# ZKTLabs/zkt-plonk

Measured on AMD Instinct MI355X. Metric: proofs/sec (withdraw, n=2^20), higher is better.
Workload: dtype u32 limbs (256-bit Montgomery); 1 GPU; full prove, WithdrawCircuit INPUTS=8 HEIGHT=64 Poseidon x5 (1019498 gates, 538 Poseidon gadgets), bn254, n=2^20, TABLE_SIZE=1024, 12 public inputs; parallelism=proofs sharded across 1 GPU(s), chained=True, distinct_witnesses=2, witness_on_device=True, table_cached=True, proof_bytes=802

## Files before the change

include/zkt_plonk.h:

```cpp
#ifndef ZKT_PLONK_H
#define ZKT_PLONK_H

#include <stddef.h>
#include <stdint.h>

#ifdef __cplusplus
extern "C" {
#endif

typedef struct zkt_ctx zkt_ctx;

enum {
    ZKT_CURVE_BN254 = 0,
    ZKT_CURVE_BLS12_381 = 1
};

enum {
    ZKT_OK = 0,
    ZKT_ERR_INVALID_ARGUMENT = 1,
    ZKT_ERR_INVALID_DOMAIN_SIZE = 2,
    ZKT_ERR_HIP = 3,
    ZKT_ERR_NO_DEVICE = 4,
    ZKT_ERR_TOO_MANY_COEFFICIENTS = 5,
    ZKT_ERR_ZERO_DENOMINATOR = 6,
    ZKT_ERR_EQUAL_CHALLENGES = 7,
    ZKT_ERR_NOT_IN_TABLE = 8,
    ZKT_ERR_QUOTIENT_TOO_SHORT = 9,
    ZKT_ERR_NOT_LOADED = 10,
    ZKT_ERR_COMM = 11
};

int zkt_ctx_create(int curve_id, int device_id, zkt_ctx** out);
void zkt_ctx_destroy(zkt_ctx* ctx);
int zkt_ctx_fork(zkt_ctx* ctx, zkt_ctx** out);
const char* zkt_last_error(const zkt_ctx* ctx);
int zkt_ctx_set_stream(zkt_ctx* ctx, void* hip_stream);
int zkt_ctx_synchronize(zkt_ctx* ctx);
int zkt_profile_enable(zkt_ctx* ctx, int on);
int zkt_profile_get(zkt_ctx* ctx, const char* name, uint64_t* calls, double* total_ms);
const char* zkt_version(void);

typedef struct {
    void* user;
    int rank;
    int world;
    int device_buffers;
    int (*all_gather)(void* user, const void* send, void* recv, size_t bytes, int on_device, void* hip_stream);
    int (*all_gather_async)(void* user, const void* d_send, void* d_recv, size_t bytes, void* hip_stream);
} zkt_comm_vtable;
#define ZKT_QUOTIENT_CHUNKS 4
int zkt_ctx_set_comm(zkt_ctx* ctx, const zkt_comm_vtable* comm);
int zkt_shard_range(size_t total, int rank, int world, size_t* lo, size_t* hi);
int zkt_comm_stats(zkt_ctx* ctx, uint64_t* calls, uint64_t* bytes_sent);
int zkt_comm_selftest(const zkt_comm_vtable* comm, const void* send, void* recv, size_t bytes);

int zkt_dev_alloc(zkt_ctx* ctx, size_t bytes, void** dptr);
int zkt_dev_free(zkt_ctx* ctx, void* dptr);
int zkt_dev_upload(zkt_ctx* ctx, void* dptr, const void* host, size_t bytes);
int zkt_dev_download(zkt_ctx* ctx, void* host, const void* dptr, size_t bytes);

int zkt_ntt(zkt_ctx* ctx, int log_n, int inverse, int coset, const uint64_t* in, size_t in_len, uint64_t* out);
int zkt_ntt_dev(zkt_ctx* ctx, int log_n, int inverse, int coset, const void* d_in, size_t in_len, void* d_out);
int zkt_ntt_class(zkt_ctx* ctx, int log_n, int log_big, int cls, const uint64_t* in, size_t in_len, uint64_t* out);
int zkt_domain_group_gen(zkt_ctx* ctx, int log_n, uint64_t* out4);

int zkt_srs_load(zkt_ctx* ctx, const uint64_t* g1_xy_mont, size_t count);
int zkt_srs_load_dev(zkt_ctx* ctx, const void* d_g1_xy_mont, size_t count);
int zkt_srs_generate(zkt_ctx* ctx, const uint64_t* tau_canonical4, size_t count);
int zkt_srs_download(zkt_ctx* ctx, size_t offset, size_t count, uint64_t* out_xy_mont);
int zkt_srs_generate_g2(int curve_id, const uint64_t* tau_canonical4, uint64_t* out_h, uint64_t* out_beta_h);
int zkt_srs_load_slice(zkt_ctx* ctx, const uint64_t* g1_xy_mont_slice, size_t offset, size_t count, size_t total);
int zkt_srs_generate_slice(zkt_ctx* ctx, const uint64_t* tau_canonical4, size_t offset, size_t count, size_t total);
int zkt_msm_g1(zkt_ctx* ctx, const uint64_t* scalars, size_t len, size_t base_offset, int scalars_montgomery,
               uint64_t* out_xy_mont, int* out_is_infinity);
int zkt_msm_g1_dev(zkt_ctx* ctx, const void* d_scalars, size_t len, size_t base_offset, int scalars_montgomery,
                   void* out_xy_mont_host);
int zkt_msm_enqueue_dev(zkt_ctx* ctx, const void* d_scalars, size_t len, size_t base_offset, int scalars_montgomery);
int zkt_msm_info(zkt_ctx* ctx, int* window_bits, int* windows, size_t* srs_count);

#define ZKT_MSM_BASES_MAX ((size_t)1 << 22)
int zkt_msm_g1_bases(zkt_ctx* ctx, const uint64_t* bases_xy_mont, const uint64_t* scalars, size_t n,
                     int scalars_montgomery, uint64_t* out_xy_mont, int* out_is_infinity);
int zkt_msm_g1_bases_dev(zkt_ctx* ctx, const void* d_bases_xy_mont, const void* d_scalars, size_t n,
                         int scalars_montgomery, uint64_t* out_xy_mont_host, int* out_is_infinity);
int zkt_msm_bases_info(zkt_ctx* ctx, size_t n, int scalars_montgomery, int* window_bits, int* windows);

#define ZKT_KZG_BATCH_MAX 32
int zkt_kzg_commit_batch(zkt_ctx* ctx, const uint64_t* const* coeffs, const size_t* lens, int k,
                         int scalars_montgomery, uint64_t* out_xy_mont, int* out_is_infinity);
int zkt_kzg_commit_batch_dev(zkt_ctx* ctx, const void* const* d_coeffs, const size_t* lens, int k,
                             int scalars_montgomery, uint64_t* out_xy_mont, int* out_is_infinity);
int zkt_kzg_open(zkt_ctx* ctx, const uint64_t* const* coeffs, const size_t* lens, int k,
                 const uint64_t* challenges_mont, const uint64_t* point_mont,
                 uint64_t* out_w_xy_mont, int* out_w_is_infinity, uint64_t* out_evals_mont);
int zkt_kzg_open_dev(zkt_ctx* ctx, const void* const* d_coeffs, const size_t* lens, int k,
                     const uint64_t* challenges_mont, const uint64_t* point_mont,
                     uint64_t* out_w_xy_mont, int* out_w_is_infinity, uint64_t* out_evals_mont);

int zkt_ctx_set_lagrange(zkt_ctx* ctx, int on);
int zkt_ctx_set_wire_elimination(zkt_ctx* ctx, int mode);
int zkt_ctx_set_quotient_route(zkt_ctx* ctx, int mode);
int zkt_ctx_set_fused_passes(zkt_ctx* ctx, int mode);
int zkt_lagrange_info(zkt_ctx* ctx, int* log_n, size_t* bases);
int zkt_commit_evals_dev(zkt_ctx* ctx, const void* d_evals, const uint64_t* blinders, int k, int path, uint64_t* out_xy_mont,
                         int* out_is_infinity);

enum {
    ZKT_TRANSCRIPT_MERLIN = 0,
    ZKT_TRANSCRIPT_ETHEREUM = 1
};
typedef struct zkt_transcript zkt_transcript;
zkt_transcript* zkt_transcript_new(int kind, const char* label);
void zkt_transcript_free(zkt_transcript* t);
void zkt_transcript_append_u64(zkt_transcript* t, const char* label, uint64_t v);
void zkt_transcript_append_scalars(zkt_transcript* t, const char* label, const uint8_t* le32, size_t count, int single);
void zkt_transcript_append_commitment(zkt_transcript* t, const char* label, const uint8_t* x_le, const uint8_t* y_le,
                                      size_t fq_bytes, int is_infinity);
void zkt_transcript_challenge_scalar(zkt_transcript* t, const char* label, int fr_bits, uint8_t out_le32[32]);
void zkt_transcript_seed(zkt_transcript* t, uint64_t circuit_size, const uint8_t* xy_le, const uint8_t* is_infinity,
                         size_t fq_bytes);
int zkt_transcript_append_message(zkt_transcript* t, const char* label, const uint8_t* msg, size_t len);
int zkt_transcript_challenge_bytes(zkt_transcript* t, const char* label, uint8_t* out, size_t len);

typedef struct {
    void* user;
    void (*append_u64)(void* user, const char* label, uint64_t v);
    void (*append_scalars)(void* user, const char* label, const uint64_t* fr_mont, size_t count, int single);
    void (*append_commitment)(void* user, const char* label, const uint64_t* g1_xy_mont, int is_infinity);
    void (*challenge_scalar)(void* user, const char* label, uint64_t* fr_mont_out4);
} zkt_transcript_vtable;

int zkt_circuit_load(zkt_ctx* ctx, int log_n, const uint64_t* const* pk_polys, const size_t* pk_lens);

int zkt_circuit_setup(zkt_ctx* ctx, int log_n, const uint64_t* const* evals, const size_t* eval_lens, int evals_on_device,
                      uint64_t* out_commitments, int* out_is_infinity);

int zkt_circuit_sigma_dev(zkt_ctx* ctx, int log_n, const uint32_t* d_w_l, const uint32_t* d_w_r, const uint32_t* d_w_o,
                          size_t n_rows, size_t n_vars, void* const* d_sigma);
int zkt_circuit_setup_wiring(zkt_ctx* ctx, int log_n, const uint64_t* const* evals, const size_t* eval_lens,
                             int evals_on_device, const uint32_t* w_l, const uint32_t* w_r, const uint32_t* w_o,
                             size_t n_rows, size_t n_vars, int wiring_on_device,
                             uint64_t* out_commitments, int* out_is_infinity);

typedef struct {
    const uint64_t* a_evals;
    const uint64_t* b_evals;
    const uint64_t* c_evals;
    size_t n_rows;
    const uint64_t* table;
    size_t table_len;
    const size_t* pi_pos;
    const uint64_t* pi_vals;
    size_t n_pi;
    const uint64_t* blinders;
    int wires_on_device;
    const uint64_t* variables;
    size_t n_vars;
    const uint32_t* w_l;
    const uint32_t* w_r;
    const uint32_t* w_o;
} zkt_prove_inputs;
#define ZKT_VARIABLE_ZERO 0xFFFFFFFFu

int zkt_prove(zkt_ctx* ctx, const zkt_prove_inputs* in, zkt_transcript* transcript, uint8_t* proof_out,
              size_t proof_cap, size_t* proof_len);
int zkt_prove_set_next(zkt_ctx* ctx, const zkt_prove_inputs* next);
int zkt_prove_with(zkt_ctx* ctx, const zkt_prove_inputs* in, const zkt_transcript_vtable* transcript,
                   uint8_t* proof_out, size_t proof_cap, size_t* proof_len);

enum {
    ZKT_CHECK_WIRING = 1
};
#define ZKT_CHECK_NONE ((uint64_t)-1)
typedef struct {
    int satisfied;
    int checked;
    uint64_t n_arithmetic;
    uint64_t first_arithmetic;
    uint64_t residual[4];
    uint64_t n_lookup;
    uint64_t first_lookup;
    uint64_t n_wiring;
// ... 359 lines not shown
```

zkt-plonk_amd/_lib.py:

```python
from __future__ import annotations

import ctypes
import os
import re
from typing import Optional

import numpy as np

_HERE = os.path.dirname(os.path.abspath(__file__))
_LIB = os.environ.get("ZKT_LIB_PATH") or os.path.join(_HERE, "libzkt_plonk_hip.so")
_HEADER = os.path.join(_HERE, "..", "include", "zkt_plonk.h")

MSM_BASES_MAX = 1 << 22
G1_DECOMPRESS_MAX = 1 << 22
VERIFY_BATCH_DEV_MAX = MSM_BASES_MAX // 24
KZG_BATCH_MAX = 32
CURVE_BN254 = 0
CURVE_BLS12_381 = 1
_CURVES = {"bn254": 0, "bls12_381": 1, "bls12-381": 1, 0: 0, 1: 1}

_lib = None


class ZktError(RuntimeError):
# ... 1643 lines not shown

    def debug_verify_batch_tree(self, items, h_g2, beta_h_g2):
        ins, trs, k, h, bh, keep = _verify_batch_args(self.curve, items, h_g2, beta_h_g2)
        n_nodes = sum(verify_tree_levels(max(k, 1)))
        nodes = np.zeros((2, n_nodes, 2 * self.fq_limbs), dtype=np.uint64)
        inf = (ctypes.c_int * (2 * n_nodes))()
        rho = np.zeros((2 * max(k, 1), 4), dtype=np.uint64)
        self.check(self._L.zkt_debug_verify_batch_tree(self._h, ins, trs, k, u64p(h), u64p(bh), u64p(nodes), inf, u64p(rho)))
        return nodes, np.array([bool(x) for x in inf]).reshape(2, n_nodes), rho[:2 * k]

    def set_verify_terms(self, mode: int = 0):
        self._L.zkt_ctx_set_verify_terms.argtypes = [ctypes.c_void_p, ctypes.c_int]
        self.check(self._L.zkt_ctx_set_verify_terms(self._h, int(mode)))

    def debug_verify_terms(self, items, rho=None, forced=None, route: int = 2):
        rc, out = _verify_terms_call(self._L.zkt_debug_verify_terms, self._h, self.curve, items, rho, forced, route)
        self.check(rc)
        return out

    def msm_bases_info(self, n: int, montgomery: bool = True):
        c, w = ctypes.c_int(0), ctypes.c_int(0)
        self.check(self._L.zkt_msm_bases_info(self._h, n, int(montgomery), ctypes.byref(c), ctypes.byref(w)))
        return dict(window_bits=c.value, windows=w.value)

    def _kzg_polys(self, polys):
        arrs = [np.ascontiguousarray(p, dtype=np.uint64).reshape(-1, 4) for p in polys]
        ptrs = (ctypes.c_void_p * max(len(arrs), 1))(*[a.ctypes.data if a.shape[0] else None for a in arrs])
        return arrs, ptrs, self._kzg_lens([a.shape[0] for a in arrs])

    @staticmethod
    def _kzg_lens(lens):
        return (ctypes.c_size_t * max(len(lens), 1))(*[int(n) for n in lens])

    def _kzg_points(self, out, inf, k):
        W = 2 * self.fq_limbs
        return [(out[j * W:(j + 1) * W].copy(), bool(inf[j])) for j in range(k)]

    def kzg_commit_batch(self, polys, montgomery: bool = True):
        arrs, ptrs, lens = self._kzg_polys(polys)
        k = len(arrs)
        out = np.zeros(max(k, 1) * 2 * self.fq_limbs, dtype=np.uint64)
        inf = (ctypes.c_int * max(k, 1))()
        self.check(self._L.zkt_kzg_commit_batch(self._h, ptrs, lens, k, int(montgomery), u64p(out), inf))
        return self._kzg_points(out, inf, k)

    def kzg_commit_batch_dev(self, d_ptrs, lens, montgomery: bool = True):
        k = len(lens)
        ptrs = (ctypes.c_void_p * max(k, 1))(*[int(d) if d else None for d in d_ptrs])
        out = np.zeros(max(k, 1) * 2 * self.fq_limbs, dtype=np.uint64)
        inf = (ctypes.c_int * max(k, 1))()
        self.check(self._L.zkt_kzg_commit_batch_dev(self._h, ptrs, self._kzg_lens(lens), k, int(montgomery), u64p(out), inf))
        return self._kzg_points(out, inf, k)

    def _kzg_open_call(self, fn, ptrs, lens, k, challenges, z, evals):
        ch = np.ascontiguousarray(challenges, dtype=np.uint64).reshape(-1, 4)
        if ch.shape[0] != k:
            raise ValueError("kzg_open: %d polynomials, %d challenges" % (k, ch.shape[0]))
        zz = np.ascontiguousarray(z, dtype=np.uint64).reshape(4)
        w = np.zeros(2 * self.fq_limbs, dtype=np.uint64)
        inf = ctypes.c_int(0)
        ev = np.zeros((max(k, 1), 4), dtype=np.uint64)
        self.check(fn(self._h, ptrs, lens, k, u64p(ch) if k else None, u64p(zz), u64p(w), ctypes.byref(inf),
                      u64p(ev) if evals else None))
        return (w, bool(inf.value)), (ev[:k].copy() if evals else None)

    def kzg_open(self, polys, challenges, z, evals: bool = True):
        arrs, ptrs, lens = self._kzg_polys(polys)
        return self._kzg_open_call(self._L.zkt_kzg_open, ptrs, lens, len(arrs), challenges, z, evals)

    def kzg_open_dev(self, d_ptrs, lens, challenges, z, evals: bool = True):
        k = len(lens)
        ptrs = (ctypes.c_void_p * max(k, 1))(*[int(d) if d else None for d in d_ptrs])
        return self._kzg_open_call(self._L.zkt_kzg_open_dev, ptrs, self._kzg_lens(lens), k, challenges, z, evals)

    def msm_info(self):
        c, w, n = ctypes.c_int(0), ctypes.c_int(0), ctypes.c_size_t(0)
        self.check(self._L.zkt_msm_info(self._h, ctypes.byref(c), ctypes.byref(w), ctypes.byref(n)))
        return dict(window_bits=c.value, windows=w.value, srs_count=n.value)

    def set_lagrange(self, on: bool = True):
        self._L.zkt_ctx_set_lagrange.argtypes = [ctypes.c_void_p, ctypes.c_int]
        self.check(self._L.zkt_ctx_set_lagrange(self._h, int(on)))

    def set_wire_elimination(self, mode: int = 1):
        self._L.zkt_ctx_set_wire_elimination.argtypes = [ctypes.c_void_p, ctypes.c_int]
        self.check(self._L.zkt_ctx_set_wire_elimination(self._h, int(mode)))

    def lagrange_info(self):
        self._L.zkt_lagrange_info.argtypes = [ctypes.c_void_p, ctypes.POINTER(ctypes.c_int), ctypes.POINTER(ctypes.c_size_t)]
        lg, nb = ctypes.c_int(0), ctypes.c_size_t(0)
        self.check(self._L.zkt_lagrange_info(self._h, ctypes.byref(lg), ctypes.byref(nb)))
        return dict(log_n=lg.value, bases=nb.value)

    def commit_evals_dev(self, d_evals: int, blinders=None, path: int = 1):
        self._L.zkt_commit_evals_dev.argtypes = [ctypes.c_void_p, ctypes.c_void_p, ctypes.POINTER(ctypes.c_uint64), ctypes.c_int,
                                                 ctypes.c_int, ctypes.POINTER(ctypes.c_uint64), ctypes.POINTER(ctypes.c_int)]
        k = 0 if blinders is None else int(np.asarray(blinders).reshape(-1, 4).shape[0])
        bl = np.ascontiguousarray(blinders, dtype=np.uint64).reshape(-1, 4) if k else None
        out = np.zeros(2 * self.fq_limbs, dtype=np.uint64)
        inf = ctypes.c_int(0)
        self.check(self._L.zkt_commit_evals_dev(self._h, ctypes.c_void_p(d_evals), u64p(bl) if k else None, k, int(path),
                                                u64p(out), ctypes.byref(inf)))
        return out, bool(inf.value)

    def circuit_load(self, log_n: int, pk_polys):
        arrs = [np.ascontiguousarray(p, dtype=np.uint64).reshape(-1, 4) for p in pk_polys]
        assert len(arrs) == 10
        ptrs = (ctypes.POINTER(ctypes.c_uint64) * 10)(*[u64p(a) if a.size else ctypes.POINTER(ctypes.c_uint64)() for a in arrs])
        lens = (ctypes.c_size_t * 10)(*[a.shape[0] for a in arrs])
        self.check(self._L.zkt_circuit_load(self._h, log_n, ptrs, lens))
        self.circuit_log_n = log_n

    def circuit_setup(self, log_n: int, evals):
        arrs = [np.ascontiguousarray(p, dtype=np.uint64).reshape(-1, 4) for p in evals]
        assert len(arrs) == 10
        ptrs = (ctypes.POINTER(ctypes.c_uint64) * 10)(*[u64p(a) if a.size else ctypes.POINTER(ctypes.c_uint64)() for a in arrs])
        lens = (ctypes.c_size_t * 10)(*[a.shape[0] for a in arrs])
        out = np.zeros((10, 2 * self.fq_limbs), dtype=np.uint64)
        inf = (ctypes.c_int * 10)()
        self.check(self._L.zkt_circuit_setup(self._h, log_n, ptrs, lens, 0, u64p(out), inf))
        self.circuit_log_n = log_n
        return out, np.array([bool(x) for x in inf])

    def circuit_sigma(self, log_n: int, d_w_l: int, d_w_r: int, d_w_o: int, n_rows: int, n_vars: int, d_sigma=None):
        n = 1 << log_n if 0 <= log_n <= 25 else 0
        own = d_sigma is None
        if own:
            d_sigma = [self.alloc(max(n, 1) * 32) for _ in range(3)]
        try:
            ptrs = (ctypes.c_void_p * 3)(*d_sigma)
            self.check(self._L.zkt_circuit_sigma_dev(self._h, log_n, ctypes.c_void_p(d_w_l), ctypes.c_void_p(d_w_r),
                                                     ctypes.c_void_p(d_w_o), n_rows, n_vars, ptrs))
            return [self.download(p, (n, 4)) for p in d_sigma] if own else None
        finally:
            if own:
                for p in d_sigma:
                    self.free(p)

    def circuit_setup_wiring(self, log_n: int, evals, w_l, w_r, w_o, n_vars: int, n_rows: int = None):
        assert len(evals) == 10
        arrs = [np.zeros((0, 4), dtype=np.uint64) if p is None else np.ascontiguousarray(p, dtype=np.uint64).reshape(-1, 4)
                for p in evals]
        ptrs = (ctypes.POINTER(ctypes.c_uint64) * 10)(*[u64p(a) if a.size else ctypes.POINTER(ctypes.c_uint64)() for a in arrs])
        lens = (ctypes.c_size_t * 10)(*[a.shape[0] for a in arrs])
        on_device = isinstance(w_l, int)
        if on_device:
            assert n_rows is not None
            w = [ctypes.c_void_p(p) for p in (w_l, w_r, w_o)]
        else:
            idx = [np.ascontiguousarray(x, dtype=np.uint32).reshape(-1) for x in (w_l, w_r, w_o)]
            assert idx[0].shape == idx[1].shape == idx[2].shape
            n_rows = idx[0].shape[0] if n_rows is None else n_rows
            w = [x.ctypes.data_as(ctypes.c_void_p) if x.size else ctypes.c_void_p() for x in idx]
        out = np.zeros((10, 2 * self.fq_limbs), dtype=np.uint64)
        inf = (ctypes.c_int * 10)()
        self.check(self._L.zkt_circuit_setup_wiring(self._h, log_n, ptrs, lens, 0, w[0], w[1], w[2], n_rows, n_vars,
                                                    int(on_device), u64p(out), inf))
        self.circuit_log_n = log_n
        return out, np.array([bool(x) for x in inf])

    def _prepare(self, wires, n_rows, table, pi_pos, pi_vals, blinders, on_device, variables=None, idx=None, keep=()):
        table = np.ascontiguousarray(table, dtype=np.uint64).reshape(-1, 4)
        pi_vals = np.ascontiguousarray(pi_vals, dtype=np.uint64).reshape(-1, 4)
        if blinders is None:
            blinders = np.zeros((0, 4), dtype=np.uint64)
        else:
# ... 295 lines not shown
```

zkt-plonk_amd/csrc/capi.hip:

```cpp
#include "ctx.hpp"

#include <cstdlib>
#include "hostinv.hpp"
#include "ec.hpp"
#include "hostec.hpp"
#include "fx_test.hpp"
#include "msm.hpp"

#include <atomic>
#include <cstring>

namespace zkt {

const char* exp_env(const char* name) {
#ifdef ZKT_EXPERIMENTS
    return getenv(name);
#else
    (void)name;
    return nullptr;
#endif
}

int set_err(zkt_ctx* c, int code, const std::string& msg) {
    if (c) c->err = msg;
// ... 163 lines not shown
    (void)hipStreamSynchronize(c->stream);
    (void)hipDeviceSynchronize();
    for (auto& kv : c->prof) {
        for (auto& pr : kv.second.pending) {
            float ms = 0.f;
            if (hipEventElapsedTime(&ms, pr.first, pr.second) == hipSuccess) kv.second.total_ms += ms;
            c->event_pool.push_back(pr.first);
            c->event_pool.push_back(pr.second);
        }
        kv.second.pending.clear();
    }
}

template <class P>
__global__ void k_fr_mul(const Fe<P>* a, const Fe<P>* b, Fe<P>* o, size_t n) {
    size_t i = (size_t)blockIdx.x * blockDim.x + threadIdx.x;
    if (i < n) fe_store<P>(o + i, fe_mul<P>(fe_load<P>(a + i), fe_load<P>(b + i)));
}

template <class P>
__global__ void k_fx_test(int op, const uint32_t* in, size_t n, uint32_t* out) {
    constexpr int W = 4 * FxP<P>::L;
    size_t i = (size_t)blockIdx.x * blockDim.x + threadIdx.x;
    if (i < n) fx_test_op<P>(op, in + i * W, out + i * W);
}
template <class Q>
__global__ void k_xyzz_test(int op, const uint32_t* in, size_t n, uint32_t* out) {
    constexpr int W = 4 * FxP<Q>::L + 1;
    size_t i = (size_t)blockIdx.x * blockDim.x + threadIdx.x;
    if (i < n) xyzz_test_op<Q>(op, in + i * 2 * W, out + i * W);
}

template <class P>
static int dump_params(uint32_t* out, size_t words) {
    const int N = P::N;
    if (words < (size_t)(3 * N + 1)) return -1;
    for (int i = 0; i < N; ++i) out[i] = P::mod(i);
    out[N] = P::INV;
    for (int i = 0; i < N; ++i) out[N + 1 + i] = P::one(i);
    for (int i = 0; i < N; ++i) out[2 * N + 1 + i] = P::r2(i);
    return N;
}

}

using namespace zkt;

extern "C" {

const char* zkt_version(void) { return "zkt-plonk_amd 0.1 (gfx950)"; }

int zkt_ctx_create(int curve_id, int device_id, zkt_ctx** out) {
    if (!out) return ZKT_ERR_INVALID_ARGUMENT;
    *out = nullptr;
    if (curve_id != ZKT_CURVE_BN254 && curve_id != ZKT_CURVE_BLS12_381) return ZKT_ERR_INVALID_ARGUMENT;
    int count = 0;
    if (hipGetDeviceCount(&count) != hipSuccess || count <= 0 || device_id < 0 || device_id >= count)
        return ZKT_ERR_NO_DEVICE;
    if (hipSetDevice(device_id) != hipSuccess) return ZKT_ERR_NO_DEVICE;
    zkt_ctx* c = new zkt_ctx(device_id);
    c->batch_off = exp_env("ZKT_MSM_NO_BATCH") != nullptr;
    c->aux_off = exp_env("ZKT_NO_AUX") != nullptr;
    if (const char* parts = exp_env("ZKT_FUSED_PARTS")) c->fused_parts = atoi(parts) & 63;
    c->curve = curve_id;
    if (hipStreamCreateWithFlags(&c->stream, hipStreamNonBlocking) != hipSuccess) {
        delete c;
        return ZKT_ERR_HIP;
    }
    c->own_stream = true;
    *out = c;
    return ZKT_OK;
}

int zkt_ctx_fork(zkt_ctx* parent, zkt_ctx** out) {
    if (!parent || !out) return ZKT_ERR_INVALID_ARGUMENT;
    *out = nullptr;
    if (parent->sharded()) return set_err(parent, ZKT_ERR_INVALID_ARGUMENT, "zkt_ctx_fork: not for a context with a communicator");
    zkt_ctx* c = nullptr;
    int rc = zkt_ctx_create(parent->curve, parent->device, &c);
    if (rc) return rc;
    (void)hipStreamSynchronize(parent->stream);
    c->is_fork = true;
    c->lagrange_off = parent->lagrange_off;
    c->wire_elim_mode = parent->wire_elim_mode;
    c->quotient_route = parent->quotient_route;
    c->fused_passes = parent->fused_passes;
    c->verify_terms_mode = parent->verify_terms_mode;
    c->fused_parts = parent->fused_parts;
    c->batch_off = parent->batch_off;
    c->aux_off = parent->aux_off;
    c->ntt_plans = parent->ntt_plans;
    if ((rc = msm_fork(c, parent)) || (rc = circuit_fork(c, parent))) {
        parent->err = c->err;
        zkt_ctx_destroy(c);
        return rc;
    }
    *out = c;
    return ZKT_OK;
}

void zkt_ctx_destroy(zkt_ctx* c) {
    if (!c) return;
    (void)hipSetDevice(c->device);
    (void)hipStreamSynchronize(c->stream);
    circuit_release(c);
    msm_release(c);
    prof_resolve(c);
    for (hipEvent_t e : c->event_pool) (void)hipEventDestroy(e);
    c->event_pool.clear();
    c->msmb.reset();
    c->kzg.reset();
    c->ntt_plans.clear();
    if (c->comm.pinned) (void)hipHostFree(c->comm.pinned);
    c->owned.clear();
    if (c->own_stream && c->stream) (void)hipStreamDestroy(c->stream);
    delete c;
}

int zkt_ctx_set_comm(zkt_ctx* c, const zkt_comm_vtable* comm) {
    if (!c) return ZKT_ERR_INVALID_ARGUMENT;
    if (int rf = refuse_if_forked(c, "zkt_ctx_set_comm")) return rf;
    if (c->is_fork && comm && comm->world > 1) return set_err(c, ZKT_ERR_INVALID_ARGUMENT, "a forked context cannot take a communicator");
    if (comm && comm->world > 1) {
        const int w = comm->world;
        if ((w != 2 && w != 4 && w != 8) || comm->rank < 0 || comm->rank >= w || !comm->all_gather)
            return set_err(c, ZKT_ERR_INVALID_ARGUMENT, "communicator: world must be 1, 2, 4 or 8 with a valid rank and callback");
    }
    (void)hipSetDevice(c->device);
    (void)hipStreamSynchronize(c->stream);
    circuit_release(c);
    msm_release(c);
    c->comm.vt = zkt_comm_vtable{};
    c->comm.vt.world = 1;
    if (comm && comm->world > 1) c->comm.vt = *comm;
    c->comm.calls = 0;
    c->comm.bytes = 0;
    return ZKT_OK;
}
int zkt_shard_range(size_t total, int rank, int world, size_t* lo, size_t* hi) {
    if (world < 1 || rank < 0 || rank >= world || !lo || !hi) return ZKT_ERR_INVALID_ARGUMENT;
    const size_t base = total / (size_t)world, rem = total % (size_t)world;
    *lo = (size_t)rank * base + ((size_t)rank < rem ? (size_t)rank : rem);
    *hi = *lo + base + ((size_t)rank < rem ? 1 : 0);
    return ZKT_OK;
}
int zkt_comm_stats(zkt_ctx* c, uint64_t* calls, uint64_t* bytes_sent) {
    if (!c || !calls || !bytes_sent) return ZKT_ERR_INVALID_ARGUMENT;
    *calls = c->comm.calls;
    *bytes_sent = c->comm.bytes;
    return ZKT_OK;
}
int zkt_comm_selftest(const zkt_comm_vtable* comm, const void* send, void* recv, size_t bytes) {
    if (!comm || !comm->all_gather || !send || !recv) return ZKT_ERR_INVALID_ARGUMENT;
    return comm->all_gather(comm->user, send, recv, bytes, 0, nullptr) ? ZKT_ERR_COMM : ZKT_OK;
}

const char* zkt_last_error(const zkt_ctx* c) { return c ? c->err.c_str() : "null context"; }

int zkt_ctx_set_stream(zkt_ctx* c, void* hip_stream) {
    if (!c) return ZKT_ERR_INVALID_ARGUMENT;
    ZKT_HIP(c, hipStreamSynchronize(c->stream));
    if (c->own_stream && c->stream) (void)hipStreamDestroy(c->stream);
    c->stream = (hipStream_t)hip_stream;
    c->own_stream = false;
    return ZKT_OK;
}

int zkt_ctx_set_lagrange(zkt_ctx* c, int on) {
    if (!c) return ZKT_ERR_INVALID_ARGUMENT;
    c->lagrange_off = !on;
    ++c->msm_epoch;
    return ZKT_OK;
}

int zkt_ctx_set_wire_elimination(zkt_ctx* c, int mode) {
    if (!c) return ZKT_ERR_INVALID_ARGUMENT;
    if (mode < 0 || mode > 2) return set_err(c, ZKT_ERR_INVALID_ARGUMENT, "mode: 0 off, 1 automatic, 2 whenever a table can be built");
    c->wire_elim_mode = mode;
    ++c->msm_epoch;
    return ZKT_OK;
}

int zkt_ctx_set_quotient_route(zkt_ctx* c, int mode) {
    if (!c) return ZKT_ERR_INVALID_ARGUMENT;
    if (mode < 0 || mode > 2) return set_err(c, ZKT_ERR_INVALID_ARGUMENT, "mode: 0 automatic, 1 three classes, 2 the whole coset");
    c->quotient_route = mode;
    return ZKT_OK;
}

int zkt_ctx_set_fused_passes(zkt_ctx* c, int mode) {
    if (!c) return ZKT_ERR_INVALID_ARGUMENT;
    if (mode < 0 || mode > 2) return set_err(c, ZKT_ERR_INVALID_ARGUMENT, "mode: 0 automatic, 1 fused, 2 one launch per step");
    c->fused_passes = mode;
    return ZKT_OK;
}

int zkt_profile_enable(zkt_ctx* c, int on) {
    if (!c) return ZKT_ERR_INVALID_ARGUMENT;
    prof_resolve(c);
    if (on) c->prof.clear();
    c->prof_on = on == 2 ? 2 : (on != 0 ? 1 : 0);
    return ZKT_OK;
}
int zkt_profile_get(zkt_ctx* c, const char* name, uint64_t* calls, double* total_ms) {
    if (!c || !name || !calls || !total_ms) return ZKT_ERR_INVALID_ARGUMENT;
    prof_resolve(c);
    std::string key(name);
    const size_t hash = key.find("#launches");
    const bool want_launches = hash != std::string::npos;
    if (want_launches) key.resize(hash);
    auto it = c->prof.find(key);
    if (it == c->prof.end()) {
        *calls = 0;
        *total_ms = 0.0;
        return ZKT_OK;
    }
    *calls = want_launches ? it->second.launches : it->second.calls;
    *total_ms = it->second.total_ms;
    return ZKT_OK;
}

int zkt_ctx_synchronize(zkt_ctx* c) {
    if (!c) return ZKT_ERR_INVALID_ARGUMENT;
    ZKT_HIP(c, hipStreamSynchronize(c->stream));
    return ZKT_OK;
}

int zkt_dev_alloc(zkt_ctx* c, size_t bytes, void** dptr) {
    if (!c || !dptr) return ZKT_ERR_INVALID_ARGUMENT;
    (void)hipSetDevice(c->device);
    return dev_alloc(c, dptr, bytes);
}
int zkt_dev_free(zkt_ctx* c, void* dptr) {
    if (!c) return ZKT_ERR_INVALID_ARGUMENT;
    ZKT_HIP(c, hipStreamSynchronize(c->stream));
    dev_free(c, dptr);
    return ZKT_OK;
}
int zkt_dev_upload(zkt_ctx* c, void* dptr, const void* host, size_t bytes) {
    if (!c || (!dptr && bytes) || (!host && bytes)) return ZKT_ERR_INVALID_ARGUMENT;
    ZKT_HIP(c, hipMemcpyAsync(dptr, host, bytes, hipMemcpyHostToDevice, c->stream));
    ZKT_HIP(c, hipStreamSynchronize(c->stream));
    return ZKT_OK;
}
int zkt_dev_download(zkt_ctx* c, void* host, const void* dptr, size_t bytes) {
    if (!c || (!dptr && bytes) || (!host && bytes)) return ZKT_ERR_INVALID_ARGUMENT;
    ZKT_HIP(c, hipMemcpyAsync(host, dptr, bytes, hipMemcpyDeviceToHost, c->stream));
    ZKT_HIP(c, hipStreamSynchronize(c->stream));
    return ZKT_OK;
}

int zkt_ntt_dev(zkt_ctx* c, int log_n, int inverse, int coset, const void* d_in, size_t in_len, void* d_out) {
    if (!c || !d_out || (!d_in && in_len)) return set_err(c, ZKT_ERR_INVALID_ARGUMENT, "null pointer");
// ... 282 lines not shown
```

zkt-plonk_amd/csrc/circuit.hpp:

```cpp
#pragma once
#include "ctx.hpp"
#include "ec.hpp"
#include "hostinv.hpp"
#include "poly.hpp"
#include "quotient_classes.hpp"
#include <cstring>

namespace zkt {

enum { PK_QM = 0, PK_QL, PK_QR, PK_QO, PK_QC, PK_S1, PK_S2, PK_S3, PK_QLOOKUP, PK_QTABLE, PK_COUNT };
enum { CS_QM = 0, CS_QL, CS_QR, CS_QO, CS_QC, CS_QLOOKUP, CS_QTABLE, CS_S1, CS_S2, CS_S3, CS_X, CS_L1, CS_COUNT };
enum { W_A = 0, W_B, W_C, W_PI, W_Z1, W_Z2, W_T, W_H1, W_H2, W_COUNT };

struct CircuitKeys {
    std::shared_ptr<DevShared> keys_mem;
    void* pk[PK_COUNT] = {};
    size_t pk_len[PK_COUNT] = {};
    void* coset[CS_COUNT] = {};
    void* sigma_ev[3] = {};
    void* q_lookup_ev = nullptr;
    void* roots = nullptr;
    uint32_t zh_inv[4][8] = {};
};
struct ClassTables {
    std::shared_ptr<DevShared> class_mem;
    void* ccoset[CS_COUNT] = {};
    bool ccoset_ready = false;
    uint32_t key_win[4][QCW][8] = {};
    uint32_t qc_gamma[4][8] = {}, qc_vinv[9][8] = {}, qc_g3[3][8] = {};
};

struct CircuitState : CircuitKeys, ClassTables {
    DevSet work;
    explicit CircuitState(int device) : work(device) {}
    int log_n = 0;
    size_t n = 0;
    int G = 1, cls = 0, log_m = 0;
    size_t m = 0;
    void* wnext[4] = {};
    void* fold = nullptr;
    void* qgather = nullptr;
    bool have[16] = {};
    void* ev[8] = {};
    void* sc[4] = {};
    void* scan_tmp = nullptr;
    void* poly[13] = {};
    void* wcos[W_COUNT] = {};
    void* qev = nullptr;
    void* lag_scalars = nullptr;
    void* lag_scalars_q[3] = {};
    void* small = nullptr;
    uint32_t* status = nullptr;
    uint32_t* lk_u32 = nullptr;
    uint32_t lk_nkeys = 0;
    std::vector<uint32_t> lk_host_keys, lk_host_sorted, lk_host_counts, lk_host_order;
    bool has_next = false, prefetch_same_table = false;
    int prefetch_stage = 0;
    uint64_t prefetch_epoch = 0;
    zkt_prove_inputs next_in{}, prefetch_in{};
    void* poly_alt[3] = {};
    uint32_t* status_alt = nullptr;
    void* lk_keys = nullptr;
    size_t lk_cap = 0;
    void* pinned = nullptr;
    hipStream_t comm_stream = nullptr;
    hipEvent_t ev_piece[ZKT_QUOTIENT_CHUNKS] = {}, ev_gathered = nullptr;
    hipStream_t aux_stream = nullptr;
    hipEvent_t ev_aux_go = nullptr, ev_aux_done = nullptr;
    void* aux_scan_tmp = nullptr;
    void* aux_pw = nullptr;
    hipStream_t copy_stream = nullptr;
    hipEvent_t ev_copy[4] = {};
    void* pinned_pi = nullptr;
    uint32_t* pi_tab = nullptr;
    void* eval_pw = nullptr;
    std::vector<uint64_t> cached_table;
    bool t_cached = false, t_coset_valid = false;
    uint64_t t_srs_generation = 0;
    uint64_t t_commit_xy[12] = {};
    bool wire_route[3] = {};
    bool wire_dense_only = false;
    int wire_elim_force = -1;
    bool use_classes = false;
    void* heads = nullptr;
    void* d_win = nullptr;
    void* pinned_win = nullptr;
    hipEvent_t ev_win = nullptr;
    bool vk_cached = false;
    uint64_t vk_srs_generation = 0;
    uint64_t vk_commits[10 * 12] = {};
    int vk_inf[10] = {};
    size_t vk_table_size = 0;
    uint32_t last_u[6][8] = {};
    bool last_u_valid = false;
};

template <class P>
struct HostF {
    using F = Fe<P>;
    static F from_words(const uint64_t* w) {
        F r;
        memcpy(r.v, w, 32);
        return r;
    }
    static void to_le_bytes(const F& mont, uint8_t out[32]) {
        F c = fe_from_mont<P>(mont);
        memcpy(out, c.v, 32);
    }
    static F from_le_bytes(const uint8_t in[32]) {
        F c;
        memcpy(c.v, in, 32);
        return fe_to_mont<P>(c);
    }
};

template <class Q>
static void fq_to_le(const Fe<Q>& mont, uint8_t* out) {
    Fe<Q> c = fe_from_mont<Q>(mont);
    memcpy(out, c.v, Q::N * 4);
}

template <class Fn>
static auto by_curve(int curve, Fn&& f) {
    return curve == ZKT_CURVE_BN254 ? f(Bn254Curve{}) : f(Bls381Curve{});
}

enum : unsigned {
    ENTRY_DOMAIN = 1u,
    ENTRY_SRS = 2u,
    ENTRY_WHOLE_KEY = 4u,
    ENTRY_WHOLE_COSET = 8u,
    ENTRY_NO_NEXT = 16u,
    ENTRY_DEVICE = 32u,
    ENTRY_WITHDRAW = 64u,
    ENTRY_WORK = ENTRY_WHOLE_COSET | ENTRY_NO_NEXT | ENTRY_DEVICE | ENTRY_WITHDRAW,
};
inline int circuit_entry(zkt_ctx* c, unsigned needs, const char* who = "") {
    if (!c->circuit)
        return set_err(c, ZKT_ERR_NOT_LOADED, needs & ENTRY_DOMAIN ? "no circuit loaded (the domain comes from it)" : "no circuit loaded (zkt_circuit_load)");
    if ((needs & ENTRY_SRS) && !c->msm) return set_err(c, ZKT_ERR_NOT_LOADED, "no SRS loaded (zkt_srs_load)");
    if ((needs & ENTRY_WHOLE_KEY) && c->sharded()) return set_err(c, ZKT_ERR_INVALID_ARGUMENT, "not available on a sharded key");
    if ((needs & ENTRY_WHOLE_COSET) && (c->sharded() || c->circuit->G != 1))
        return set_err(c, ZKT_ERR_INVALID_ARGUMENT, std::string(who) + ": a sharded context holds one class of every coset and a slice of the key; use an unsharded one");
    if ((needs & ENTRY_NO_NEXT) && c->circuit->has_next) return set_err(c, ZKT_ERR_INVALID_ARGUMENT, std::string(who) + ": a next proof is announced");
    if (needs & ENTRY_DEVICE) (void)hipSetDevice(c->device);
    if (needs & ENTRY_WITHDRAW) c->circuit->prefetch_stage = 0;
    return ZKT_OK;
}

int circuit_key_coset(zkt_ctx* c, CircuitState& S, const void* poly, size_t len, void* out);
int circuit_commit_keys(zkt_ctx* c, CircuitState& S, const size_t* lens, uint64_t* out_commitments, int* out_is_inf);
int circuit_key_lens(zkt_ctx* c, const CircuitState& S, size_t* lens10);
int check_sharded_key(zkt_ctx* c);

template <class R>
static void circuit_zh4(int log_n, Fe<R> out[4]) {
    const size_t n = (size_t)1 << log_n;
    const Fe<R> one = fe_one<R>(), g = fe_from_u32<R>(R::GENERATOR), w4n = root_of_unity<R>(log_n + 2);
    const Fe<R> w4 = fe_pow_u64<R>(w4n, (uint64_t)n);
    Fe<R> cur = fe_pow_u64<R>(g, (uint64_t)n);
    for (int j = 0; j < 4; ++j) {
        out[j] = fe_sub<R>(cur, one);
        cur = fe_mul<R>(cur, w4);
// ... 38 lines not shown
```

zkt-plonk_amd/csrc/circuit_steps.hip:

```cpp
#include "circuit.hpp"
#include "msm.hpp"

namespace zkt {

template <class R>
static void debug_quotient_classes_host_t(int log_n, const uint64_t* windows, const uint64_t* challenges, uint64_t* out_u,
                                          uint64_t* out_consts) {
    typedef Fe<R> F;
    const QuotientClassConsts<R> q = quotient_class_consts<R>(log_n);
    for (int k = 0; k < 4; ++k) memcpy(out_consts + 4 * k, q.gamma[k].v, 32);
    for (int k = 0; k < 9; ++k) memcpy(out_consts + 4 * (4 + k), q.vinv[k].v, 32);
    for (int k = 0; k < 3; ++k) memcpy(out_consts + 4 * (13 + k), q.g3[k].v, 32);
    const uint32_t* w = (const uint32_t*)windows;
    QuotientWindows W{};
    const uint32_t** slot[10] = {&W.a, &W.b, &W.c, &W.z1, &W.z2, &W.t, &W.sigma1, &W.sigma2, &W.sigma3, &W.q_lookup};
    for (int k = 0; k < 10; ++k) *slot[k] = w + (size_t)k * QCW * 8;
    F alpha, beta, delta, u[6];
    memcpy(alpha.v, challenges, 32);
    memcpy(beta.v, challenges + 4, 32);
    memcpy(delta.v, challenges + 8, 32);
    quotient_top_coefficients<R>(log_n, W, alpha, beta, delta, u);
    for (int e = 0; e < 6; ++e) memcpy(out_u + 4 * e, u[e].v, 32);
}

}

using namespace zkt;

extern "C" {

int zkt_debug_quotient_top(zkt_ctx* c, uint64_t* out_u, int* out_on_classes) {
    if (!c || !out_u) return set_err(c, ZKT_ERR_INVALID_ARGUMENT, "null pointer");
    if (int rc = circuit_entry(c, 0)) return rc;
    const CircuitState& S = *c->circuit;
    if (out_on_classes) *out_on_classes = S.use_classes ? 1 : 0;
    memcpy(out_u, S.last_u, sizeof(S.last_u));
    return ZKT_OK;
}

int zkt_debug_quotient_coeffs(zkt_ctx* c, uint64_t* out, size_t count) {
    if (!c || !out) return set_err(c, ZKT_ERR_INVALID_ARGUMENT, "null pointer");
    if (int rc = circuit_entry(c, ENTRY_DEVICE)) return rc;
    const CircuitState& S = *c->circuit;
    if (count > 4 * S.n) return set_err(c, ZKT_ERR_INVALID_ARGUMENT, "the quotient vector holds 4n elements");
    ZKT_HIP(c, hipStreamSynchronize(c->stream));
    ZKT_HIP(c, hipMemcpy(out, S.qev, count * 32, hipMemcpyDeviceToHost));
    return ZKT_OK;
}

int zkt_debug_quotient_classes_host(int curve, int log_n, const uint64_t* windows, const uint64_t* challenges, uint64_t* out_u,
                                    uint64_t* out_consts) {
    if (!windows || !challenges || !out_u || !out_consts) return ZKT_ERR_INVALID_ARGUMENT;
    if (curve != ZKT_CURVE_BN254 && curve != ZKT_CURVE_BLS12_381) return ZKT_ERR_INVALID_ARGUMENT;
    return by_curve(curve, [&](auto C) {
        using R = typename decltype(C)::Fr;
        if (log_n < 3 || log_n + 2 > R::TWO_ADICITY) return (int)ZKT_ERR_INVALID_DOMAIN_SIZE;
        debug_quotient_classes_host_t<R>(log_n, windows, challenges, out_u, out_consts);
        return (int)ZKT_OK;
    });
}

int zkt_lagrange_info(zkt_ctx* c, int* log_n, size_t* bases) {
    if (!c) return ZKT_ERR_INVALID_ARGUMENT;
    const bool ready = c->circuit && lagrange_ready(c, c->circuit->log_n) && !c->lagrange_off;
    if (log_n) *log_n = ready ? c->circuit->log_n : -1;
    if (bases) *bases = ready ? lagrange_bases(c) : 0;
    return ZKT_OK;
}

int zkt_commit_evals_dev(zkt_ctx* c, const void* d_evals, const uint64_t* blinders, int k, int path, uint64_t* out_xy,
                         int* out_is_infinity) {
    if (!c || !d_evals || !out_xy || (k > 0 && !blinders)) return set_err(c, ZKT_ERR_INVALID_ARGUMENT, "null pointer");
    if (k < 0 || k > 3) return set_err(c, ZKT_ERR_INVALID_ARGUMENT, "0 .. 3 blinders");
    if (int rc0 = circuit_entry(c, ENTRY_DOMAIN | ENTRY_SRS | ENTRY_WHOLE_KEY | ENTRY_DEVICE | ENTRY_WITHDRAW)) return rc0;
    CircuitState& S = *c->circuit;
    const size_t n = S.n;
    int rc;
    if (path == 1) {
        if ((rc = lagrange_ensure(c, S.log_n))) return rc;
        if (!lagrange_ready(c, S.log_n)) return set_err(c, ZKT_ERR_NOT_LOADED, "the key is too short for the Lagrange-basis table");
    } else if (path != 0) {
        return set_err(c, ZKT_ERR_INVALID_ARGUMENT, "path: 0 coefficients, 1 Lagrange basis");
    }
    uint32_t* d_len = S.status + 8 + 12;
    void* d_bl = (char*)S.lag_scalars + (n + 8) * 32;
    void* poly = S.poly[12];
    ZKT_HIP(c, hipMemsetAsync(d_len, 0, 4, c->stream));
    if (k) ZKT_HIP(c, hipMemcpyAsync(d_bl, blinders, (size_t)k * 32, hipMemcpyHostToDevice, c->stream));
    if ((rc = ntt_run(c, S.log_n, 1, 0, d_evals, n, poly))) return rc;
    if (c->fused(4)) {
        const TrimBlindSpec tb{poly, d_bl, d_len, k};
        if ((rc = poly_trim_blind(c, &tb, 1, n, 8))) return rc;
    } else {
        if ((rc = poly_trim_len(c, poly, n, d_len, (char*)poly + n * 32, 8))) return rc;
        if (k && (rc = poly_add_blinders(c, poly, d_len, d_bl, k, n + 8))) return rc;
    }
    if (path == 0) return msm_g1_dev(c, poly, n + (size_t)k, 0, 1, out_xy, out_is_infinity);
    if ((rc = lagrange_scalars(c, d_evals, n, d_len, d_bl, k, S.roots, S.lag_scalars))) return rc;
    if ((rc = msm_begin(c, S.lag_scalars, n + (size_t)k, 0, 1, 0, 1))) return rc;
    uint64_t xy[12] = {};
    if ((rc = msm_end(c, 0, xy))) return rc;
    const size_t words = c->curve == ZKT_CURVE_BN254 ? 8 : 12;
    memcpy(out_xy, xy, words * 8);
    if (out_is_infinity) {
        bool any = false;
        for (size_t i = 0; i < words; ++i) any = any || xy[i] != 0;
        *out_is_infinity = any ? 0 : 1;
    }
    return ZKT_OK;
}

int zkt_debug_quotient(zkt_ctx* c, const uint64_t* challenges, const uint64_t* const* wit, const uint64_t* pi_pos,
                       const uint64_t* pi_vals, size_t n_pi, uint64_t* out) {
    if (!c || !challenges || !wit || !out || (n_pi && (!pi_pos || !pi_vals)))
        return set_err(c, ZKT_ERR_INVALID_ARGUMENT, "null pointer");
    if (int rc0 = circuit_entry(c, ENTRY_DEVICE)) return rc0;
    CircuitState& S = *c->circuit;
    if (S.G != 1) return set_err(c, ZKT_ERR_INVALID_ARGUMENT, "zkt_debug_quotient: whole-coset circuits only");
    if (n_pi > (size_t)QUOTIENT_PI_DIRECT_MAX) return set_err(c, ZKT_ERR_INVALID_ARGUMENT, "too many direct public inputs");
    for (size_t i = 0; i < n_pi; ++i)
        if (pi_pos[i] >= S.n) return set_err(c, ZKT_ERR_INVALID_ARGUMENT, "public input position out of range");
    const size_t bytes = 4 * S.n * 32;
    DevSet tmp(c->device);
    void* d[W_COUNT] = {};
    void* d_out = nullptr;
    uint32_t* d_tab = nullptr;
    int rc = ZKT_OK;
    for (int k = 0; k < W_COUNT && !rc; ++k) {
        if (k == W_PI && n_pi) continue;
        if (!wit[k]) rc = set_err(c, ZKT_ERR_INVALID_ARGUMENT, "null witness coset");
        else if (!(rc = tmp.alloc(c, &d[k], bytes)) && hipMemcpy(d[k], wit[k], bytes, hipMemcpyHostToDevice) != hipSuccess)
            rc = set_err(c, ZKT_ERR_HIP, "copy of a witness coset failed");
    }
    if (!rc) rc = tmp.alloc(c, &d_out, bytes);
    if (!rc && n_pi) {
        std::vector<uint32_t> tab(10 * n_pi);
        by_curve(c->curve, [&](auto C) { pi_rows<typename decltype(C)::Fr>(pi_pos, pi_vals, n_pi, 1, tab.data()); });
        if (!(rc = tmp.alloc(c, (void**)&d_tab, tab.size() * 4)) &&
            hipMemcpy(d_tab, tab.data(), tab.size() * 4, hipMemcpyHostToDevice) != hipSuccess)
            rc = set_err(c, ZKT_ERR_HIP, "copy of the public-input rows failed");
    }
    if (!rc) {
        QuotientArgs q = quotient_args(S, d, challenges, challenges + 4, challenges + 8, challenges + 12, challenges + 16);
        q.out = d_out;
        q.n4 = 4 * S.n;
        q.pi_tab = n_pi ? d_tab : nullptr;
        q.n_pi_direct = (uint32_t)n_pi;
        rc = quotient_pointwise(c, q);
        if (!rc && hipStreamSynchronize(c->stream) != hipSuccess) rc = set_err(c, ZKT_ERR_HIP, "quotient kernel failed");
        if (!rc && hipMemcpy(out, d_out, bytes, hipMemcpyDeviceToHost) != hipSuccess) rc = set_err(c, ZKT_ERR_HIP, "copy back failed");
    }
    return rc;
}

int zkt_debug_eval_lincomb(zkt_ctx* c, const uint64_t* const* polys, const size_t* lens, int k, const uint64_t* points,
                           const uint64_t* scalars, uint64_t* out_evals, uint64_t* out_lincomb, size_t out_len) {
    if (!c || !polys || !lens || !points || !scalars || !out_evals || !out_lincomb) return set_err(c, ZKT_ERR_INVALID_ARGUMENT, "null pointer");
    if (int rc0 = circuit_entry(c, ENTRY_DEVICE | ENTRY_WITHDRAW)) return rc0;
    CircuitState& S = *c->circuit;
    const size_t cap = S.n + 8;
    if (k < 1 || k > 12 || out_len < 1 || out_len > cap) return set_err(c, ZKT_ERR_INVALID_ARGUMENT, "1 .. 12 polynomials, out_len <= n + 8");
    for (int j = 0; j < k; ++j)
        if (!polys[j] || lens[j] < 1 || lens[j] > cap) return set_err(c, ZKT_ERR_INVALID_ARGUMENT, "1 .. n + 8 coefficients each");
    EvalArgs ea{};
    LinCombArgs lc{};
    ea.count = k;
    lc.nterms = k;
    for (int j = 0; j < k; ++j) {
        ZKT_HIP(c, hipMemcpyAsync(S.poly[j], polys[j], lens[j] * 32, hipMemcpyHostToDevice, c->stream));
        ea.poly[j] = lc.poly[j] = S.poly[j];
        ea.len[j] = lc.len[j] = lens[j];
        memcpy(ea.point[j], points + 4 * j, 32);
        memcpy(lc.scalar[j], scalars + 4 * j, 32);
    }
    void* d_partials = (char*)S.small + 64 * 32;
    void* d_results = (char*)S.small + 32 * 32;
    int rc = poly_eval_many(c, ea, d_partials, d_results, S.eval_pw);
    if (rc) return rc;
    if ((rc = poly_lincomb(c, lc, S.sc[0], out_len))) return rc;
    ZKT_HIP(c, hipMemcpyAsync(out_evals, d_results, (size_t)k * 32, hipMemcpyDeviceToHost, c->stream));
    ZKT_HIP(c, hipMemcpyAsync(out_lincomb, S.sc[0], out_len * 32, hipMemcpyDeviceToHost, c->stream));
    ZKT_HIP(c, hipStreamSynchronize(c->stream));
    return ZKT_OK;
}
// ... 25 lines not shown
```

zkt-plonk_amd/csrc/ctx.hpp:

```cpp
#pragma once
#include <hip/hip_runtime.h>
#include <stdint.h>
#include <stddef.h>
#include <map>
#include <string>
#include <tuple>
#include <vector>
#include <memory>

#include "../../include/zkt_plonk.h"
#include "fp.hpp"
#include "fx.hpp"
#include "ntt.hpp"

namespace zkt {

struct MsmState;
struct MsmBasesState;
struct KzgState;
struct CircuitState;

struct DevSet {
    const int device;
    std::vector<std::pair<void*, size_t>> mem;
    std::vector<void*> host;
    std::vector<hipStream_t> streams;
    std::vector<hipEvent_t> events;
    explicit DevSet(int dev) : device(dev) {}
    DevSet(const DevSet&) = delete;
    DevSet& operator=(const DevSet&) = delete;
    ~DevSet() { clear(); }
    void clear();
    int alloc(zkt_ctx* c, void** p, size_t bytes);
    void release(void* p);
    int pinned(zkt_ctx* c, void** p, size_t bytes, unsigned flags = 0);
    int stream(zkt_ctx* c, hipStream_t* s);
    int event(zkt_ctx* c, hipEvent_t* e);
};
struct DevBuf {
    void* p = nullptr;
    size_t bytes = 0;
};

}

struct zkt_ctx {
    int curve = 0;
    const int device;
    explicit zkt_ctx(int dev) : device(dev), owned(dev) {}
    hipStream_t stream = nullptr;
    bool own_stream = false;
    std::string err;

    std::map<std::tuple<int, int, int, int>, std::shared_ptr<void>> ntt_plans;
    int ntt_split_npass = 0;
    int ntt_split_log_r[3] = {0, 0, 0};
    zkt::DevBuf ntt_scratch, io_a, io_b;
    zkt::DevBuf check_scratch;
    zkt::DevBuf verify_scratch;

    int prof_on = 0;
    struct ProfSlot {
        std::vector<std::pair<hipEvent_t, hipEvent_t>> pending;
        double total_ms = 0.0;
        uint64_t calls = 0;
        uint64_t launches = 0;
    };
    std::map<std::string, ProfSlot> prof;
    std::vector<hipEvent_t> event_pool;

    struct Comm {
        zkt_comm_vtable vt{};
        void* pinned = nullptr;
        size_t pinned_bytes = 0;
        uint64_t calls = 0, bytes = 0;
    } comm;
    bool sharded() const { return comm.vt.world > 1; }

    std::shared_ptr<zkt::MsmState> msm;
    std::shared_ptr<zkt::MsmBasesState> msmb;
    std::shared_ptr<zkt::KzgState> kzg;
    size_t srs_check_chunk = 0;
    size_t store_chunk = 0;
    uint64_t msm_epoch = 0;
    uint64_t srs_generation = 0;
    bool is_fork = false;
    bool aux_off = false;
    bool batch_off = false;
    bool lagrange_off = false;
    int wire_elim_mode = 1;
    int quotient_route = 0;
    int verify_terms_mode = 0;
    int fused_passes = 0;
    int fused_parts = 63;
    bool fused(int part) const { return fused_passes != 2 && (fused_parts & part); }
    std::shared_ptr<zkt::CircuitState> circuit;
    zkt::DevSet owned;
};

namespace zkt {

const char* exp_env(const char* name);

int set_err(zkt_ctx* c, int code, const std::string& msg);
int refuse_if_forked(zkt_ctx* c, const char* what);
int hip_fail(zkt_ctx* c, hipError_t e, const char* what);

#define ZKT_HIP(c, call)                                        \
    do {                                                        \
        hipError_t _e = (call);                                 \
        if (_e != hipSuccess) return zkt::hip_fail((c), _e, #call); \
    } while (0)

struct ProfScope {
    zkt_ctx* c;
    zkt_ctx::ProfSlot* slot = nullptr;
    hipEvent_t e0 = nullptr, e1 = nullptr;
    hipStream_t stream = nullptr;
    uint64_t count = 1;
    ProfScope(zkt_ctx* ctx, const char* name, hipStream_t on_stream = nullptr, uint64_t units = 1);
    ~ProfScope();
};

int comm_all_gather_host(zkt_ctx* c, const void* send, void* recv, size_t bytes);
int comm_all_gather_dev(zkt_ctx* c, const void* d_send, void* d_recv, size_t bytes);
bool comm_async_available(const zkt_ctx* c);
int comm_all_gather_async(zkt_ctx* c, const void* d_send, void* d_recv, size_t bytes, hipStream_t st);

int grow(zkt_ctx* c, DevBuf& b, size_t bytes, DevSet* in = nullptr);
inline int dev_alloc(zkt_ctx* c, void** p, size_t bytes) { return c->owned.alloc(c, p, bytes); }
inline void dev_free(zkt_ctx* c, void* p) { c->owned.release(p); }

struct DevShared : DevSet {
    using DevSet::DevSet;
    std::shared_ptr<DevShared> from;
};
inline std::shared_ptr<DevShared> dev_shared_reader(const std::shared_ptr<DevShared>& of) {
    if (!of) return nullptr;
    auto r = std::make_shared<DevShared>(of->device);
    r->from = of;
    return r;
}
inline bool dev_shared_has_readers(const std::shared_ptr<DevShared>& m) { return m && m.use_count() > 1; }

template <class P>
Fe<P> root_of_unity(int log_n);
int ntt_run(zkt_ctx* c, int log_n, int inverse, int coset, const void* d_in, size_t in_len, void* d_out);
int ntt_run_batch(zkt_ctx* c, int log_n, int inverse, int coset, int nb, const void* const* d_in, const size_t* in_len,
                  void* const* d_out, const void* d_head = nullptr);
int ntt_fold_heads(zkt_ctx* c, int nb, const void* const* d_in, size_t n, const uint32_t* gammas, void* d_out);
int ntt_run_classes(zkt_ctx* c, int log_n, int inverse, const int codes[3], int nb, const void* const* d_in, const size_t* in_len,
                    void* const* d_out, size_t in_stride, size_t out_stride, const void* d_head = nullptr);
int ntt_class_code(int log_big, int cls);
int ntt_force_split(zkt_ctx* c, int npass, const int* log_r);
int ntt_run_class(zkt_ctx* c, int log_n, int log_big, int cls, const void* d_in, size_t in_len, void* d_out, void* d_fold);

void circuit_release(zkt_ctx* c);
int circuit_fork(zkt_ctx* child, const zkt_ctx* parent);
bool circuit_tables_have_readers(const zkt_ctx* c);

}
```

zkt-plonk_amd/csrc/msm.hip:

```cpp
#include "ctx.hpp"
#include "ec.hpp"
#include "ecx.hpp"
#include "hostec.hpp"
#include "msm.hpp"

#include <algorithm>
#include <functional>
#include <type_traits>
#include <cstdlib>
#include <cstring>

namespace zkt {

template <class C>
__global__ void k_srs_generate(Affine<typename C::Fq>* out, size_t count, Fe<typename C::Fr> tau_mont,
                               Affine<typename C::Fq> g, size_t first) {
    using Q = typename C::Fq;
    using R = typename C::Fr;
    size_t i = (size_t)blockIdx.x * blockDim.x + threadIdx.x;
    if (i >= count) return;
    Fe<R> s = fe_from_mont<R>(fe_from_mont<R>(fe_pow_u64<R>(tau_mont, (uint64_t)(first + i))));
    Xyzz<Q> acc = xyzz_identity<Q>();
    bool started = false;
#pragma unroll 1
// ... 720 lines not shown
    Xyzz<Q>* buckets = (Xyzz<Q>*)tb.buckets[blockIdx.y];
    const uint32_t* heavy = tb.heavy[blockIdx.y];
    const uint32_t chunk = tb.params[blockIdx.y][0];
    __shared__ Xyzz<Q> wsum[4];
    const uint32_t nheavy = heavy[0];
    const uint32_t base = offsets[1];
    for (uint32_t h = blockIdx.x; h < nheavy; h += gridDim.x) {
        const uint32_t b = heavy[1 + h];
        const uint32_t s = offsets[b], e = offsets[b + 1];
        const uint32_t t0 = (s - base) / chunk, t1 = (e - 1 - base) / chunk;
        XyzzX<Q> acc = xx_identity<Q>();
        for (uint32_t t = t0 + threadIdx.x; t <= t1; t += 256) acc = xx_add<Q, MSM_TAIL_INL>(acc, xx_load_raw<Q>(pieces + (size_t)t + b));
        acc = block_sum_256<Q, MSM_TAIL_INL>(acc, wsum);
        if (threadIdx.x == 0) xx_store<Q>(buckets + b, acc);
    }
}

template <class Q, bool MSM_TAIL_INL>
ZKT_D XyzzX<Q> wave_sum(XyzzX<Q> acc) {
#pragma unroll 1
    for (int d = 32; d >= 1; d >>= 1) {
        XyzzX<Q> o = xx_shfl_down<Q>(acc, d);
        if ((threadIdx.x & 63) + d >= 64) o = xx_identity<Q>();
        acc = xx_add<Q, MSM_TAIL_INL>(acc, o);
    }
    return acc;
}

struct MsmTailWindows {
    struct Strided {
        char* base;
        size_t stride;
        __device__ void* operator[](uint32_t y) const { return base + (size_t)y * stride; }
    };
    Strided buckets, rowcol, partials;
};

template <class C, bool MSM_TAIL_INL, class TB = MsmTailBatch>
__global__ __launch_bounds__(256) void k_msm_rowcol(uint32_t q1, uint32_t q2, TB tb) {
    using Q = typename C::Fq;
    const Xyzz<Q>* buckets = (const Xyzz<Q>*)tb.buckets[blockIdx.y];
    Xyzz<Q>* rc = (Xyzz<Q>*)tb.rowcol[blockIdx.y];
    const uint32_t NI = 1u << q1, NJ = 1u << q2;
    const uint32_t lane = threadIdx.x & 63u;
    const uint32_t w = blockIdx.x * 4u + (threadIdx.x >> 6);
    if (w >= NI + NJ) return;
    XyzzX<Q> acc = xx_identity<Q>();
    if (w < NI) {
        for (uint32_t j = lane; j < NJ; j += 64) acc = xx_add<Q, MSM_TAIL_INL>(acc, xx_load<Q>(buckets + (size_t)w * NJ + j));
    } else {
        const uint32_t j = w - NI;
        for (uint32_t i = lane; i < NI; i += 64) acc = xx_add<Q, MSM_TAIL_INL>(acc, xx_load<Q>(buckets + (size_t)i * NJ + j));
    }
    acc = wave_sum<Q, MSM_TAIL_INL>(acc);
    if (lane == 0) xx_store<Q>(rc + w, acc);
}

template <class C, bool MSM_TAIL_INL, class TB = MsmTailBatch>
__global__ __launch_bounds__(64) void k_msm_weighted_rows(uint32_t q1, uint32_t q2, uint32_t B, TB tb) {
    using Q = typename C::Fq;
    const Xyzz<Q>* rc = (const Xyzz<Q>*)tb.rowcol[blockIdx.y];
    const Xyzz<Q>* top_bucket = (const Xyzz<Q>*)tb.buckets[blockIdx.y] + B;
    Xyzz<Q>* partials = (Xyzz<Q>*)tb.partials[blockIdx.y];
    const uint32_t NI = 1u << q1, NJ = 1u << q2;
    const uint32_t lane = threadIdx.x & 63u;
    const uint32_t y = blockIdx.x;
    XyzzX<Q> acc = xx_identity<Q>();
    if (y == q1 + q2) {
        if (lane == 0) acc = xx_load<Q>(top_bucket);
    } else {
        const bool col = y < q2;
        const uint32_t k = col ? y : y - q2, low = (1u << k) - 1u;
        const uint32_t cnt = (col ? NJ : NI) >> 1;
        const Xyzz<Q>* src = col ? rc + NI : rc;
        for (uint32_t q = lane; q < cnt; q += 64) {
            const uint32_t idx = ((q & ~low) << 1) | (1u << k) | (q & low);
            acc = xx_add<Q, MSM_TAIL_INL>(acc, xx_load<Q>(src + idx));
        }
    }
    acc = wave_sum<Q, MSM_TAIL_INL>(acc);
    if (lane == 0) xx_store_ark<Q>(partials + y, acc);
}

template <class C>
__global__ void k_srs_to_fx(Affine<typename C::Fq>* table, size_t total) {
    using Q = typename C::Fq;
    size_t i = (size_t)blockIdx.x * blockDim.x + threadIdx.x;
    if (i >= total) return;
    Affine<Q> a = aff_load<Q>(table + i);
    if (aff_is_inf<Q>(a)) return;
    a.x = fx_pack<Q>(fx_cond_sub_p<Q>(fx_from_ark<Q>(a.x)));
    a.y = fx_pack<Q>(fx_cond_sub_p<Q>(fx_from_ark<Q>(a.y)));
    aff_store<Q>(table + i, a);
}

static int msm_rows(int c) { return c - 1; }

template <class C, bool VB = false>
static auto msm_pick_bin_count(int dig) -> decltype(&k_msm_bin_count<C, 0, VB>) {
    if constexpr (VB) {
        return k_msm_bin_count<C, 0, true>;
    } else {
        switch (dig) {
            case 1: return k_msm_bin_count<C, 1>;
            case 2: return k_msm_bin_count<C, 2>;
            case 3: return k_msm_bin_count<C, 3>;
            case 4: return k_msm_bin_count<C, 4>;
            case 5: return k_msm_bin_count<C, 5>;
            default: return k_msm_bin_count<C, 0>;
        }
    }
}
template <class C, class PF, bool VB = false>
static auto msm_pick_bin_scatter(int dig) -> decltype(&k_msm_bin_scatter<C, PF, 0, VB>) {
    if constexpr (VB) {
        return k_msm_bin_scatter<C, PF, 0, true>;
    } else {
        switch (dig) {
            case 1: return k_msm_bin_scatter<C, PF, 1>;
            case 2: return k_msm_bin_scatter<C, PF, 2>;
            case 3: return k_msm_bin_scatter<C, PF, 3>;
            case 4: return k_msm_bin_scatter<C, PF, 4>;
            case 5: return k_msm_bin_scatter<C, PF, 5>;
            default: return k_msm_bin_scatter<C, PF, 0>;
        }
    }
}

static int floor_log2(size_t x) {
    int l = 0;
    while ((x >> (l + 1)) != 0) ++l;
    return l;
}

static int msm_plan(zkt_ctx* c, int total, int cb, size_t points, bool own_buckets, MsmPlan& P) {
    P = MsmPlan{};
    const int W = (total + cb - 1) / cb;
    if (W > (int)sizeof(P.win.width)) return set_err(c, ZKT_ERR_INVALID_ARGUMENT, "msm_g1_bases: too many windows");
    const int lo = total / W, rem = total % W;
    P.W = P.win.W = W;
    int pos = 0;
    for (int w = 0; w < W; ++w) {
        P.win.width[w] = (uint8_t)(lo + (w < rem ? 1 : 0));
        P.win.start[w] = (uint16_t)pos;
        pos += P.win.width[w];
    }
    P.c = lo + (rem ? 1 : 0);
    P.dig = own_buckets ? 0 : msm_digit_layout(P.win, total);
    P.Bw = 1u << (P.c - 1);
    P.keys = own_buckets ? (uint32_t)W * P.Bw : P.Bw;
    const size_t m = (size_t)W * points;
    if (!own_buckets && m >= ((size_t)1 << 31))
        return set_err(c, ZKT_ERR_INVALID_ARGUMENT, "SRS too large for 31-bit table indices");
    {
        const size_t idx_max = (own_buckets ? points : m) - 1;
        int idx_bits = 1;
        while (idx_max >> idx_bits) ++idx_bits;
        int lb = 31 - idx_bits;
        if (lb > MSM_BIN_LB_MAX) lb = MSM_BIN_LB_MAX;
        P.packed = lb >= 4 && ((P.keys >> lb) + 1) < (uint32_t)MSM_MAX_NB1;
        P.lb = P.packed ? (uint32_t)lb : (uint32_t)MSM_BIN_LB_MAX;
        if (!P.packed && ((P.keys >> P.lb) + 1) >= (uint32_t)MSM_MAX_NB1) {
            P.lb = MSM_BIN_LB_WIDE;
            P.lcols = MSM_BIN_LB_WIDE;
        }
    }
    P.nb1 = (P.keys >> P.lb) + 1;
    if (P.nb1 >= (uint32_t)MSM_MAX_NB1 || m >= ((size_t)1 << 31))
        return set_err(c, ZKT_ERR_INVALID_ARGUMENT,
                       own_buckets ? "msm_g1_bases: digit layout outside the sort's range" : "msm: too many level-1 bins");
    P.l1_scalars = ((uint32_t)MSM_L1_CAP / (uint32_t)W) & ~63u;
    if (P.l1_scalars > 1024u) P.l1_scalars = 1024u;
    P.l2_items = (uint32_t)(m / MSM_L2_TILE + P.nb1);
    return ZKT_OK;
}

template <class C, bool VB>
static int msm_scatter_lds_cap(zkt_ctx* c, bool packed, int dig) {
    const int lds = (int)(((3 * (uint32_t)MSM_MAX_NB1 + 3) & ~3u) * 4 + MSM_L1_CAP * (packed ? 4 : 8));
// ... 35 lines not shown
    auto st = std::make_shared<MsmState>(c->device);
    struct Drain {
        zkt_ctx* c;
        ~Drain() { if (!c->msm) (void)hipStreamSynchronize(c->stream); }
    } drain{c};
    st->count = count;
    int lg = floor_log2(count ? count : 1);
    int cb = lg - 2;
    if (cb < 8) cb = 8;
    if (lg <= 20) {
        if (cb > 18) cb = 18;
        if (Q::N == 12) {
            if (lg == 20) cb = 19;
            else if (lg == 19) cb = 18;
            else if (lg == 17) cb = 16;
        } else if (lg >= 17) {
            cb = 17;
        }
    } else if (cb > 20) {
        cb = 20;
    }
    if (const char* e = exp_env("ZKT_MSM_CBITS")) {
        const int f = atoi(e);
        if (f >= 8 && f <= MSM_MAX_Y) cb = f;
    }
    int rc = msm_plan(c, R::BITS + 1, cb, count, false, st->plan);
    if (rc) return rc;
    const MsmPlan& P = st->plan;
    if (share) {
        st->table = share->table;
        st->table_mem = dev_shared_reader(share->table_mem);
        static_cast<LagrangeTable&>(*st) = *share;
        st->lag_mem = dev_shared_reader(share->lag_mem);
        if (share->wb.built && !share->wb.stale) {
            st->wb = share->wb;
            st->wb.mem = dev_shared_reader(share->wb.mem);
        }
        st->slice_off = share->slice_off;
        st->total = share->total;
    } else {
        st->table_mem = std::make_shared<DevShared>(c->device);
        if ((rc = st->table_mem->alloc(c, &st->table, (size_t)P.W * count * sizeof(Affine<Q>)))) return rc;
    }
    size_t m = (size_t)P.W * count;
    constexpr size_t NB = MSM_BATCH;
    auto up = [](size_t x) { return (x + 63) & ~(size_t)63; };
    st->strides.s_vals = up(m);
    st->strides.s_pairs_bytes = up(m) * 8;
    if ((rc = st->work.alloc(c, (void**)&st->vals2, NB * st->strides.s_vals * 4))) return rc;
    if ((rc = st->work.alloc(c, &st->pairs, NB * st->strides.s_pairs_bytes))) return rc;
    const size_t max_blk = (count + P.l1_scalars - 1) / P.l1_scalars;
    st->strides.s_bin_offs = up((size_t)P.nb1 * max_blk + 1);
    st->strides.s_bin_aux = up((size_t)P.nb1 * max_blk / MSM_SCAN_TILE + 4);
    st->strides.s_bin = up((size_t)P.nb1 + 1);
    st->strides.s_tile_desc = up(P.l2_items);
    st->strides.s_cnt = up((size_t)P.l2_items << P.lcols);
    if ((rc = st->work.alloc(c, (void**)&st->bin_offs, NB * st->strides.s_bin_offs * 4))) return rc;
    if ((rc = st->work.alloc(c, (void**)&st->bin_aux, NB * st->strides.s_bin_aux * 4))) return rc;
    if ((rc = st->work.alloc(c, (void**)&st->bin_start, NB * st->strides.s_bin * 4))) return rc;
    if ((rc = st->work.alloc(c, (void**)&st->tile_start, NB * st->strides.s_bin * 4))) return rc;
    if ((rc = st->work.alloc(c, &st->tile_desc, NB * st->strides.s_tile_desc * 8))) return rc;
    if ((rc = st->work.alloc(c, (void**)&st->cnt2, NB * st->strides.s_cnt * 4))) return rc;
    if ((rc = st->work.alloc(c, (void**)&st->pos2, NB * st->strides.s_cnt * 4))) return rc;
    if ((rc = msm_scatter_lds_cap<C, false>(c, P.packed, P.dig))) return rc;
    static_assert(MsmState::SLOTS == 11, "per-slot arrays are sized for 11 slots");
    for (int i = 0; i < MsmState::SLOTS; ++i) {
        if ((rc = st->work.alloc(c, (void**)&st->offsets[i], (((size_t)P.nb1 << P.lb) + 2) * 4))) return rc;
        if ((rc = st->work.alloc(c, (void**)&st->heavy[i], ((size_t)P.keys + 2) * 4))) return rc;
        if ((rc = st->work.alloc(c, (void**)&st->params[i], 16))) return rc;
    }
    if ((rc = msm_acc_setup<C>(c, &st->acc_threads, &st->acc_lds))) return rc;
    size_t max_chunks = std::min(m, st->acc_threads) + 1;
    for (int i = 0; i < MsmState::SLOTS; ++i)
        if ((rc = st->work.alloc(c, &st->pieces[i], (max_chunks + P.keys + 2) * sizeof(XyzzRaw<Q>)))) return rc;
    st->strides.s_chunk = up(max_chunks + 2);
    if ((rc = st->work.alloc(c, (void**)&st->chunk_bucket, NB * st->strides.s_chunk * 4))) return rc;
    if ((rc = st->work.stream(c, &st->side))) return rc;
    for (int i = 0; i < MsmState::SLOTS; ++i) {
        if ((rc = st->work.alloc(c, &st->buckets[i], ((size_t)P.keys + 1) * sizeof(Xyzz<Q>)))) return rc;
        {
            const int q = P.c - 1, q2 = q / 2, q1 = q - q2;
            if ((rc = st->work.alloc(c, &st->rowcol[i], (((size_t)1 << q1) + ((size_t)1 << q2)) * sizeof(Xyzz<Q>)))) return rc;
        }
        if ((rc = st->work.pinned(c, &st->host_result[i], (size_t)(MSM_MAX_Y + 1) * MSM_R2_BLOCKS * sizeof(Xyzz<Q>), hipHostMallocMapped))) return rc;
        ZKT_HIP(c, hipHostGetDevicePointer(&st->host_result_dev[i], st->host_result[i], 0));
        if ((rc = st->work.event(c, &st->ev_main[i]))) return rc;
        if ((rc = st->work.event(c, &st->ev_done[i]))) return rc;
    }
    st->defer_tails = count <= MSM_DEFER_MAX;
    if (const char* e = exp_env("ZKT_MSM_DEFER")) st->defer_tails = atoi(e) != 0;
    c->msm = st;
    ++c->msm_epoch;
    ++c->srs_generation;
    return ZKT_OK;
}

template <class C>
static int table_finish(zkt_ctx* c, void* table, size_t count) {
    using Q = typename C::Fq;
    MsmState& st = *c->msm;
    unsigned blocks = (unsigned)((count + 127) / 128);
    hipLaunchKernelGGL(k_srs_windows<C>, dim3(blocks), dim3(128), 0, c->stream, (Affine<Q>*)table, count, st.plan.win);
    ZKT_HIP(c, hipGetLastError());
    const size_t total = (size_t)st.plan.W * count;
    hipLaunchKernelGGL(k_srs_to_fx<C>, dim3((unsigned)((total + 255) / 256)), dim3(256), 0, c->stream,
                       (Affine<Q>*)table, total);
    ZKT_HIP(c, hipGetLastError());
    ZKT_HIP(c, hipStreamSynchronize(c->stream));
    return ZKT_OK;
}
template <class C>
static int srs_finish(zkt_ctx* c) {
    return table_finish<C>(c, c->msm->table, c->msm->count);
}
int msm_fork(zkt_ctx* child, const zkt_ctx* parent) {
    msm_release(child);
    if (!parent->msm) return ZKT_OK;
    int rc = parent->curve == ZKT_CURVE_BN254 ? msm_setup<Bn254Curve>(child, parent->msm->count, parent->msm.get())
                                               : msm_setup<Bls381Curve>(child, parent->msm->count, parent->msm.get());
    if (rc) return rc;
    child->srs_generation = parent->srs_generation;
    return ZKT_OK;
}
int msm_table_finish(zkt_ctx* c, void* table, size_t count) {
    if (c->curve == ZKT_CURVE_BN254) return table_finish<Bn254Curve>(c, table, count);
    return table_finish<Bls381Curve>(c, table, count);
}

void msm_release(zkt_ctx* c) {
    if (!c->msm) return;
    (void)hipStreamSynchronize(c->stream);
    (void)hipStreamSynchronize(c->msm->side);
    wire_bases_drop(c);
    c->msm.reset();
}
bool msm_tables_have_readers(const zkt_ctx* c) {
    return c->msm && (dev_shared_has_readers(c->msm->table_mem) || dev_shared_has_readers(c->msm->lag_mem) ||
                      dev_shared_has_readers(c->msm->wb.mem));
}

template <class C>
static int srs_load_t(zkt_ctx* c, const void* src, size_t count, bool src_on_device, size_t slice_off = 0, size_t total = 0) {
    using Q = typename C::Fq;
    if (count == 0) return set_err(c, ZKT_ERR_INVALID_ARGUMENT, "empty SRS");
    if (int rf = refuse_if_forked(c, "loading a key")) return rf;
    msm_release(c);
    int rc = msm_setup<C>(c, count);
    if (rc) return rc;
    c->msm->slice_off = slice_off;
    c->msm->total = total ? total : count;
    ZKT_HIP(c, hipMemcpyAsync(c->msm->table, src, count * sizeof(Affine<Q>),
                              src_on_device ? hipMemcpyDeviceToDevice : hipMemcpyHostToDevice, c->stream));
    {
        using R = typename C::Fr;
        Fe<R> raw_one = fe_zero<R>();
        raw_one.v[0] = 1u;
        const Fe<R> rinv = fe_from_mont<R>(raw_one);
        hipLaunchKernelGGL((k_srs_scale<C, false>), dim3((unsigned)((count + 127) / 128)), dim3(128), 0, c->stream,
                           (const Affine<Q>*)c->msm->table, (Affine<Q>*)c->msm->table, count, rinv);
        ZKT_HIP(c, hipGetLastError());
    }
    return srs_finish<C>(c);
}

template <class C>
static Affine<typename C::Fq> generator_mont();
template <>
Affine<Bn254Fq> generator_mont<Bn254Curve>() {
    Affine<Bn254Fq> g;
    g.x = fe_from_u32<Bn254Fq>(1);
    g.y = fe_from_u32<Bn254Fq>(2);
    return g;
}
// ... 125 lines not shown
        auto kc2 = P.lcols == 8 ? k_msm_l2_count<PairWide, 8> : k_msm_l2_count<PairWide, 10>;
        hipLaunchKernelGGL(kc2, dim3(items, ky), dim3(256), 0, c->stream, (const uint2*)wk.pairs, P.nb1, P.lb, wk.tile_start,
                           tile_desc, wk.cnt2, bt);
    }
    {
        auto ksc = P.lcols == 8 ? k_msm_l2_scan<8> : k_msm_l2_scan<10>;
        hipLaunchKernelGGL(ksc, dim3(P.nb1, ky), dim3(256), 0, c->stream, wk.cnt2, wk.pos2, wk.bin_start, wk.tile_start, P.keys,
                           P.lb, wk.chunk_bucket, bt);
    }
    if (P.packed) {
        hipLaunchKernelGGL((k_msm_l2_scatter<PairPacked, 8>), dim3(items, ky), dim3(MSM_L2S_THREADS), 0, c->stream,
                           (const uint32_t*)wk.pairs, P.nb1, P.lb, wk.tile_start, tile_desc, wk.cnt2, wk.pos2, wk.vals, bt);
    } else {
        auto kss = P.lcols == 8 ? k_msm_l2_scatter<PairWide, 8> : k_msm_l2_scatter<PairWide, 10>;
        hipLaunchKernelGGL(kss, dim3(items, ky), dim3(MSM_L2S_THREADS), 0, c->stream, (const uint2*)wk.pairs, P.nb1, P.lb,
                           wk.tile_start, tile_desc, wk.cnt2, wk.pos2, wk.vals, bt);
    }
    ZKT_HIP(c, hipGetLastError());
    return ZKT_OK;
}

template <class C>
static int msm_launch_accumulate(zkt_ctx* c, const MsmPlan& P, const uint32_t* vals, const uint32_t* chunk_bucket, const MsmBatch& bt,
                                 size_t n, size_t acc_threads, size_t acc_lds) {
    const uint32_t max_chunks = (uint32_t)std::min((size_t)P.W * n, acc_threads);
    hipLaunchKernelGGL(k_msm_accumulate<C>, dim3((max_chunks + 255) / 256, 1), dim3(256), acc_lds, c->stream, vals, P.keys,
                       chunk_bucket, bt);
    ZKT_HIP(c, hipGetLastError());
    return ZKT_OK;
}

template <class C>
static int msm_enqueue_batch(zkt_ctx* c, int k, const void* const* d_scalars, const size_t* ns, const size_t* base_offs, int mont,
                             const int* slots, const int* tbls) {
    MsmState& st = *c->msm;
    if (k < 1 || k > MSM_BATCH) return set_err(c, ZKT_ERR_INVALID_ARGUMENT, "msm batch size");
    ++c->msm_epoch;
    for (int j = 0; j < k; ++j)
        for (int w = 0; w < st.n_tail_wait; ++w)
            if (st.tail_wait[w] == slots[j])
                if (int rc0 = msm_launch_tails<C>(c)) return rc0;
    if (st.n_tail_wait + k > MSM_TAIL_BATCH)
        if (int rc0 = msm_launch_tails<C>(c)) return rc0;
    MsmBatch bt = st.strides;
    bool all_lag = true;
    for (int j = 0; j < k; ++j) all_lag = all_lag && tbls[j] != 0;
    size_t n_max = 0;
    for (int j = 0; j < MSM_BATCH; ++j) {
        const int jj = j < k ? j : 0;
        const int slot = slots[jj];
        if (j < k && st.pending[slot]) ZKT_HIP(c, hipStreamWaitEvent(c->stream, st.ev_done[slot], 0));
        bt.scalars[j] = d_scalars[jj];
        bt.n[j] = ns[jj];
        bt.base_off[j] = base_offs[jj];
        bt.table[j] = st.tbl_table(tbls[jj]);
        bt.tcount[j] = st.tbl_count(tbls[jj]);
        bt.heavy[j] = st.heavy[slot];
        bt.params[j] = st.params[slot];
        bt.offsets[j] = st.offsets[slot];
        bt.pieces[j] = st.pieces[slot];
        if (j < k) n_max = std::max(n_max, ns[jj]);
    }
    {
    ProfScope prof_all(c, all_lag ? "msm_lag_main" : "msm_main", nullptr, (uint64_t)k);
    const MsmWork wk{st.bin_offs, st.bin_aux, st.bin_start, st.tile_start, st.tile_desc, st.cnt2, st.pos2, st.pairs, st.vals2,
                     st.chunk_bucket};
    if (int rc = msm_launch_grouping<C, false>(c, st.plan, wk, bt, mont, n_max, (unsigned)k, st.acc_threads, st.defer_tails))
        return rc;
    for (int j = 0; j < k; ++j) {
        MsmBatch one = bt;
        one.offsets[0] = bt.offsets[j];
        one.pieces[0] = bt.pieces[j];
        one.params[0] = bt.params[j];
        one.table[0] = bt.table[j];
        {
            ProfScope prof_acc(c, tbls[j] ? "msm_lag_accumulate" : "msm_accumulate");
            if (int rc = msm_launch_accumulate<C>(c, st.plan, st.vals2 + (size_t)j * st.strides.s_vals,
                                                  st.chunk_bucket + (size_t)j * st.strides.s_chunk, one, ns[j], st.acc_threads, st.acc_lds))
                return rc;
        }
        ZKT_HIP(c, hipEventRecord(st.ev_main[slots[j]], c->stream));
        st.tail_wait[st.n_tail_wait++] = slots[j];
        st.pending[slots[j]] = true;
        if (st.defer_tails && st.n_tail_wait < MSM_TAIL_BATCH) continue;
        if (int rc = msm_launch_tails<C>(c)) return rc;
    }
    }
    return ZKT_OK;
}

template <class C>
static int msm_enqueue(zkt_ctx* c, const void* d_scalars, size_t n, size_t base_off, int mont, int slot = 0, int tbl = 0) {
    return msm_enqueue_batch<C>(c, 1, &d_scalars, &n, &base_off, mont, &slot, &tbl);
}

template <class Q>
static Xyzz<Q> msm_host_finish(const MsmState& st, int slot) {
    const int ny = msm_rows(st.plan.c);
    int exps[MSM_MAX_Y + 1];
    for (int y = 0; y <= ny; ++y) exps[y] = y;
    return hostec::weighted_row_sum<Q>((const Xyzz<Q>*)st.host_result[slot], ny + 1, MSM_R2_BLOCKS, exps);
}

template <class C>
static int msm_collect(zkt_ctx* c, int slot, Affine<typename C::Fq>* out) {
    using Q = typename C::Fq;
    MsmState& st = *c->msm;
    if (int rc0 = msm_launch_tails<C>(c)) return rc0;
    ZKT_HIP(c, hipEventSynchronize(st.ev_done[slot]));
    st.pending[slot] = false;
    *out = xyzz_to_affine_host<Q>(msm_host_finish<Q>(st, slot));
    return ZKT_OK;
}

template <class C>
static int msm_collect_sharded(zkt_ctx* c, const int* slots, const bool* have, int k, Affine<typename C::Fq>* out) {
    using Q = typename C::Fq;
    MsmState& st = *c->msm;
    const int world = c->comm.vt.world;
    std::vector<Xyzz<Q>> send(k), recv((size_t)k * world);
    if (int rc0 = msm_launch_tails<C>(c)) return rc0;
    for (int j = 0; j < k; ++j) {
        if (have[j]) {
            ZKT_HIP(c, hipEventSynchronize(st.ev_done[slots[j]]));
            st.pending[slots[j]] = false;
            send[j] = msm_host_finish<Q>(st, slots[j]);
        } else {
            send[j] = xyzz_identity<Q>();
        }
    }
    int rc = comm_all_gather_host(c, send.data(), recv.data(), (size_t)k * sizeof(Xyzz<Q>));
    if (rc) return rc;
    for (int j = 0; j < k; ++j) {
        Xyzz<Q> acc = xyzz_identity<Q>();
        for (int r = 0; r < world; ++r) acc = xyzz_add<Q>(acc, recv[(size_t)r * k + j]);
        out[j] = xyzz_to_affine_host<Q>(acc);
    }
    return ZKT_OK;
}

template <class C>
static int msm_run_t(zkt_ctx* c, const void* d_scalars, size_t n, size_t base_off, int mont, uint64_t* out_xy,
                     int* out_inf) {
    using Q = typename C::Fq;
    if (!c->msm) return set_err(c, ZKT_ERR_NOT_LOADED, "no SRS loaded (zkt_srs_load)");
    MsmState& st = *c->msm;
    if (base_off > st.count || n > st.count - base_off)
        return set_err(c, ZKT_ERR_TOO_MANY_COEFFICIENTS, "TooManyCoefficients: polynomial longer than the committer key");
    Affine<Q> res;
    if (n == 0) {
        res.x = fe_zero<Q>();
        res.y = fe_zero<Q>();
    } else {
        int rc = msm_enqueue<C>(c, d_scalars, n, base_off, mont, 0);
        if (rc) return rc;
        if ((rc = msm_collect<C>(c, 0, &res))) return rc;
    }
    memcpy(out_xy, res.x.v, Q::N * 4);
    memcpy(out_xy + Q::N / 2, res.y.v, Q::N * 4);
    if (out_inf) *out_inf = aff_is_inf<Q>(res) ? 1 : 0;
    return ZKT_OK;
}

int msm_begin(zkt_ctx* c, const void* d_scalars, size_t n, size_t base_off, int mont, int slot, int tbl) {
    if (!c->msm) return set_err(c, ZKT_ERR_NOT_LOADED, "no SRS loaded (zkt_srs_load)");
    if (slot < 0 || slot >= MsmState::SLOTS) return set_err(c, ZKT_ERR_INVALID_ARGUMENT, "bad MSM slot");
    if (tbl < 0 || tbl > MSM_TBL_WIRE + 2) return set_err(c, ZKT_ERR_INVALID_ARGUMENT, "bad MSM base table");
    if (tbl && !c->msm->tbl_table(tbl)) return set_err(c, ZKT_ERR_NOT_LOADED, "no Lagrange-basis table built");
    const size_t cnt = c->msm->tbl_count(tbl);
    if (n == 0 || base_off > cnt || n > cnt - base_off)
        return set_err(c, ZKT_ERR_TOO_MANY_COEFFICIENTS, "TooManyCoefficients: polynomial longer than the committer key");
    if (c->curve == ZKT_CURVE_BN254) return msm_enqueue<Bn254Curve>(c, d_scalars, n, base_off, mont, slot, tbl);
    return msm_enqueue<Bls381Curve>(c, d_scalars, n, base_off, mont, slot, tbl);
}
int msm_begin_batch(zkt_ctx* c, int k, const void* const* d_scalars, const size_t* ns, int mont, const int* slots, const int* tbls) {
    if (!c->msm) return set_err(c, ZKT_ERR_NOT_LOADED, "no SRS loaded (zkt_srs_load)");
    if (k < 1 || k > MSM_BATCH) return set_err(c, ZKT_ERR_INVALID_ARGUMENT, "msm batch size");
    size_t offs[MSM_BATCH] = {};
    for (int j = 0; j < k; ++j) {
        if (slots[j] < 0 || slots[j] >= MsmState::SLOTS) return set_err(c, ZKT_ERR_INVALID_ARGUMENT, "bad MSM slot");
        for (int i = 0; i < j; ++i)
            if (slots[i] == slots[j]) return set_err(c, ZKT_ERR_INVALID_ARGUMENT, "msm batch: slots must differ");
        if (tbls[j] < 0 || tbls[j] > MSM_TBL_WIRE + 2) return set_err(c, ZKT_ERR_INVALID_ARGUMENT, "bad MSM base table");
        if (tbls[j] && !c->msm->tbl_table(tbls[j])) return set_err(c, ZKT_ERR_NOT_LOADED, "no Lagrange-basis table built");
        if (ns[j] == 0 || ns[j] > c->msm->tbl_count(tbls[j]))
            return set_err(c, ZKT_ERR_TOO_MANY_COEFFICIENTS, "TooManyCoefficients: polynomial longer than the committer key");
    }
    if (c->curve == ZKT_CURVE_BN254) return msm_enqueue_batch<Bn254Curve>(c, k, d_scalars, ns, offs, mont, slots, tbls);
    return msm_enqueue_batch<Bls381Curve>(c, k, d_scalars, ns, offs, mont, slots, tbls);
}
bool msm_defers_tails(const zkt_ctx* c) { return c->msm && c->msm->defer_tails; }
bool msm_batches_grouping(const zkt_ctx* c) {
    if (!c->msm) return false;
    const size_t n = c->msm->count;
    if (const char* e = exp_env("ZKT_MSM_BATCH_MAX_LOG")) return n <= ((size_t)1 << atoi(e)) + 64;
    return n <= MSM_DEFER_MAX || (n > ((size_t)1 << 17) + 64 && n <= ((size_t)1 << 18) + 64);
}
int msm_flush_tails(zkt_ctx* c) {
    if (!c->msm) return ZKT_OK;
    if (c->curve == ZKT_CURVE_BN254) return msm_launch_tails<Bn254Curve>(c);
    return msm_launch_tails<Bls381Curve>(c);
}
int msm_begin_many(zkt_ctx* c, int k, const void* const* d_scalars, const size_t* ns, int mont, const int* slots, const int* tbls,
                   bool grouped, const std::function<int(int)>& ready) {
    for (int at = 0; at < k;) {
        const int kk = grouped ? std::min(MSM_BATCH, k - at) : 1;
        for (int j = at; j < at + kk && ready; ++j)
            if (int rc = ready(j)) return rc;
        const int rc = grouped ? msm_begin_batch(c, kk, d_scalars + at, ns + at, mont, slots + at, tbls + at)
                               : msm_begin(c, d_scalars[at], ns[at], 0, mont, slots[at], tbls[at]);
        if (rc) return rc;
        at += kk;
    }
    return msm_flush_tails(c);
}
int msm_end(zkt_ctx* c, int slot, uint64_t* out_xy) {
    if (c->curve == ZKT_CURVE_BN254) {
        Affine<Bn254Fq> a;
        int rc = msm_collect<Bn254Curve>(c, slot, &a);
        if (rc) return rc;
        memcpy(out_xy, a.x.v, 32);
        memcpy(out_xy + 4, a.y.v, 32);
        return ZKT_OK;
    }
    Affine<Bls381Fq> a;
    int rc = msm_collect<Bls381Curve>(c, slot, &a);
    if (rc) return rc;
    memcpy(out_xy, a.x.v, 48);
    memcpy(out_xy + 6, a.y.v, 48);
    return ZKT_OK;
}

int msm_end_sharded(zkt_ctx* c, const int* slots, const bool* have, int k, uint64_t* out_xy ) {
    if (c->curve == ZKT_CURVE_BN254) {
        std::vector<Affine<Bn254Fq>> a(k);
        int rc = msm_collect_sharded<Bn254Curve>(c, slots, have, k, a.data());
        if (rc) return rc;
        for (int j = 0; j < k; ++j) {
            memcpy(out_xy + 12 * j, a[j].x.v, 32);
            memcpy(out_xy + 12 * j + 4, a[j].y.v, 32);
        }
        return ZKT_OK;
    }
    std::vector<Affine<Bls381Fq>> a(k);
    int rc = msm_collect_sharded<Bls381Curve>(c, slots, have, k, a.data());
    if (rc) return rc;
    for (int j = 0; j < k; ++j) {
        memcpy(out_xy + 12 * j, a[j].x.v, 48);
        memcpy(out_xy + 12 * j + 6, a[j].y.v, 48);
    }
    return ZKT_OK;
}
void msm_slice(zkt_ctx* c, size_t* off, size_t* count, size_t* total) {
    *off = c->msm ? c->msm->slice_off : 0;
    *count = c->msm ? c->msm->count : 0;
    *total = c->msm ? c->msm->total : 0;
}

int msm_g1_dev(zkt_ctx* c, const void* d_scalars, size_t n, size_t base_off, int mont, uint64_t* out_xy, int* out_inf) {
    if (c->curve == ZKT_CURVE_BN254) return msm_run_t<Bn254Curve>(c, d_scalars, n, base_off, mont, out_xy, out_inf);
    return msm_run_t<Bls381Curve>(c, d_scalars, n, base_off, mont, out_xy, out_inf);
}
int msm_enqueue_only(zkt_ctx* c, const void* d_scalars, size_t n, size_t base_off, int mont) {
    if (!c->msm) return set_err(c, ZKT_ERR_NOT_LOADED, "no SRS loaded (zkt_srs_load)");
    if (base_off > c->msm->count || n > c->msm->count - base_off || n == 0)
        return set_err(c, ZKT_ERR_TOO_MANY_COEFFICIENTS, "TooManyCoefficients");
    if (c->curve == ZKT_CURVE_BN254) return msm_enqueue<Bn254Curve>(c, d_scalars, n, base_off, mont);
    return msm_enqueue<Bls381Curve>(c, d_scalars, n, base_off, mont);
}
int srs_load(zkt_ctx* c, const void* src, size_t count, bool on_device, size_t slice_off, size_t total) {
    if (c->curve == ZKT_CURVE_BN254) return srs_load_t<Bn254Curve>(c, src, count, on_device, slice_off, total);
    return srs_load_t<Bls381Curve>(c, src, count, on_device, slice_off, total);
}
int srs_generate(zkt_ctx* c, const uint64_t* tau4, size_t count, size_t slice_off, size_t total) {
    if (c->curve == ZKT_CURVE_BN254) return srs_generate_t<Bn254Curve>(c, tau4, count, slice_off, total);
    return srs_generate_t<Bls381Curve>(c, tau4, count, slice_off, total);
}
template <class C>
static int srs_download_t(zkt_ctx* c, size_t offset, size_t count, uint64_t* out) {
    using Q = typename C::Fq;
    using R = typename C::Fr;
    if (count == 0) return ZKT_OK;
    DevSet set(c->device);
    void* tmp = nullptr;
    int rc = set.alloc(c, &tmp, count * sizeof(Affine<Q>));
    if (rc) return rc;
    const Fe<R> r_canon = fe_one<R>();
    hipLaunchKernelGGL((k_srs_scale<C, true>), dim3((unsigned)((count + 127) / 128)), dim3(128), 0, c->stream,
                       (const Affine<Q>*)c->msm->table + offset, (Affine<Q>*)tmp, count, r_canon);
    hipError_t e = hipGetLastError();
    if (e == hipSuccess) e = hipMemcpyAsync(out, tmp, count * sizeof(Affine<Q>), hipMemcpyDeviceToHost, c->stream);
    if (e == hipSuccess) e = hipStreamSynchronize(c->stream);
    return e == hipSuccess ? ZKT_OK : hip_fail(c, e, "srs_download");
}

int srs_download(zkt_ctx* c, size_t offset, size_t count, uint64_t* out) {
    if (!c->msm) return set_err(c, ZKT_ERR_NOT_LOADED, "no SRS loaded");
    if (offset > c->msm->count || count > c->msm->count - offset) return set_err(c, ZKT_ERR_INVALID_ARGUMENT, "range");
    if (c->curve == ZKT_CURVE_BN254) return srs_download_t<Bn254Curve>(c, offset, count, out);
    return srs_download_t<Bls381Curve>(c, offset, count, out);
}
static int msm_bases_cbits(size_t n, int curve) {
    const int lg = floor_log2(n ? n : 1);
    int cb = lg - 4 < 8 ? 8 : lg - 4;
    if (curve == ZKT_CURVE_BN254) {
        if (lg >= 22) cb = 16;
        else if (lg >= 16) cb = 15;
    } else {
        if (lg >= 20) cb = 16;
// ... 253 lines not shown
```

zkt-plonk_amd/csrc/msm.hpp:

```cpp
#pragma once
#include "ctx.hpp"

#include <functional>

namespace zkt {

constexpr int MSM_CHUNK_MIN = 16;
constexpr int MSM_R2_BLOCKS = 1;
constexpr int MSM_MAX_Y = 24;

struct MsmWindows {
    int W;
    uint8_t width[40];
    uint16_t start[40];
};

struct MsmPlan {
    MsmWindows win{};
    int W = 0, c = 0;
    int dig = 0;
    uint32_t Bw = 0;
    uint32_t keys = 0;
    uint32_t lb = 8;
    int lcols = 8;
    bool packed = false;
    uint32_t nb1 = 0;
    uint32_t l1_scalars = 0;
    uint32_t l2_items = 0;
};

constexpr int MSM_BATCH = 3;
struct MsmBatch {
    const void* scalars[MSM_BATCH];
    uint64_t n[MSM_BATCH];
    uint64_t base_off[MSM_BATCH];
    const void* table[MSM_BATCH];
    uint64_t tcount[MSM_BATCH];
    uint32_t* heavy[MSM_BATCH];
    uint32_t* params[MSM_BATCH];
    uint32_t* offsets[MSM_BATCH];
    void* pieces[MSM_BATCH];
    uint64_t s_bin_offs, s_bin_aux, s_bin, s_tile_desc, s_cnt, s_pairs_bytes, s_vals, s_chunk;
    uint32_t vb_stride;
};

constexpr int MSM_TAIL_BATCH = 6;
struct MsmTailBatch {
    const uint32_t* offsets[MSM_TAIL_BATCH];
    const uint32_t* params[MSM_TAIL_BATCH];
    const void* pieces[MSM_TAIL_BATCH];
    void* buckets[MSM_TAIL_BATCH];
    uint32_t* heavy[MSM_TAIL_BATCH];
    void* rowcol[MSM_TAIL_BATCH];
    void* partials[MSM_TAIL_BATCH];
};

constexpr int MSM_HEAVY = 32;
constexpr int MSM_HEAVY_BLOCKS = 64;

struct WireBases {
    std::shared_ptr<DevShared> mem;
    void* table[3] = {};
    uint32_t* u[3] = {};
    size_t cnt[3] = {};
    bool use[3] = {};
    bool elim[3] = {};
    bool has_c[3] = {};
    bool elim_wanted = false;
    std::vector<size_t> pi_pos;
    bool built = false;
    bool stale = false;
    const void* w[3] = {};
    size_t n_rows = 0, n_vars = 0;
    int log_n = -1;
    uint64_t srs_generation = 0;
    uint64_t digest[2] = {};
};
constexpr int MSM_TBL_WIRE = 2;

struct LagrangeTable {
    std::shared_ptr<DevShared> lag_mem;
    void* table2 = nullptr;
    size_t count2 = 0;
    int lag_log_n = -1;
    bool lag_failed = false;
};

struct MsmState : LagrangeTable {
    DevSet work;
    explicit MsmState(int device) : work(device) {}
    size_t count = 0;
    size_t slice_off = 0, total = 0;
    MsmPlan plan;
    uint32_t* heavy[11] = {};
    std::shared_ptr<DevShared> table_mem;
    void* table = nullptr;
    WireBases wb;
    DevBuf wb_scalars[3];
    uint64_t* wb_dig = nullptr;
    uint64_t* wb_pin = nullptr;
    const void* tbl_table(int tbl) const { return tbl >= MSM_TBL_WIRE ? wb.table[tbl - MSM_TBL_WIRE] : tbl ? table2 : table; }
    size_t tbl_count(int tbl) const {
        return tbl >= MSM_TBL_WIRE ? wb.cnt[tbl - MSM_TBL_WIRE] + (wb.has_c[tbl - MSM_TBL_WIRE] ? 1 : 0) + 2 : tbl ? count2 : count;
    }
    uint32_t* params[11] = {};
    uint32_t* vals2 = nullptr;
    void* pairs = nullptr;
    uint32_t* bin_offs = nullptr;
    uint32_t* bin_aux = nullptr;
    uint32_t *bin_start = nullptr, *tile_start = nullptr;
    void* tile_desc = nullptr;
    uint32_t *cnt2 = nullptr, *pos2 = nullptr;
    uint32_t* chunk_bucket = nullptr;
    MsmBatch strides{};
    uint32_t* offsets[11] = {};
    void* pieces[11] = {};
    static constexpr int SLOTS = 11;
    void* buckets[SLOTS] = {};
    void* rowcol[SLOTS] = {};
    void* host_result[SLOTS] = {};
    void* host_result_dev[SLOTS] = {};
    size_t acc_lds = 0;
    size_t acc_threads = 196608;
    hipStream_t side = nullptr;
    hipEvent_t ev_main[SLOTS] = {}, ev_done[SLOTS] = {};
    bool pending[SLOTS] = {};
    bool defer_tails = false;
    int tail_wait[SLOTS] = {};
    int n_tail_wait = 0;
};

struct MsmBasesState {
    DevSet mem;
    explicit MsmBasesState(int device) : mem(device) {}
    DevBuf bases;
    DevBuf scalars;
    DevBuf vals, pairs, bin_offs, bin_aux, bin_start, tile_start, tile_desc, cnt2, pos2, chunk_bucket;
    DevBuf offsets, heavy, params, pieces, buckets, rowcol;
    DevBuf check_points, check_status;
    void* partials = nullptr;
    void* partials_dev = nullptr;
    size_t acc_lds = 0, acc_threads = 0;
};

constexpr size_t MSM_DEFER_MAX = ((size_t)1 << 16) + 64;
constexpr size_t MSM_TAIL_INL_MAX = ((size_t)1 << 18) + 64;

int srs_load(zkt_ctx* c, const void* src, size_t count, bool on_device, size_t slice_off = 0, size_t total = 0);
int srs_generate(zkt_ctx* c, const uint64_t* tau4, size_t count, size_t slice_off = 0, size_t total = 0);
void msm_release(zkt_ctx* c);
bool msm_tables_have_readers(const zkt_ctx* c);
int msm_table_finish(zkt_ctx* c, void* table, size_t count);
int msm_fork(zkt_ctx* child, const zkt_ctx* parent);
void msm_slice(zkt_ctx* c, size_t* off, size_t* count, size_t* total);
int msm_g1_dev(zkt_ctx* c, const void* d_scalars, size_t n, size_t base_off, int mont, uint64_t* out_xy, int* out_inf);
int msm_bases(zkt_ctx* c, const void* bases, bool bases_on_device, const void* scalars, bool scalars_on_device, size_t n, int mont,
              uint64_t* out_xy, int* out_inf);
int msm_bases_scratch(zkt_ctx* c, MsmBasesState** out);
int msm_begin(zkt_ctx* c, const void* d_scalars, size_t n, size_t base_off, int mont, int slot, int tbl = 0);
int msm_begin_batch(zkt_ctx* c, int k, const void* const* d_scalars, const size_t* ns, int mont, const int* slots, const int* tbls);
int msm_begin_many(zkt_ctx* c, int k, const void* const* d_scalars, const size_t* ns, int mont, const int* slots, const int* tbls,
                   bool grouped, const std::function<int(int)>& ready = {});
int msm_end(zkt_ctx* c, int slot, uint64_t* out_xy);
int msm_end_sharded(zkt_ctx* c, const int* slots, const bool* have, int k, uint64_t* out_xy );
int msm_flush_tails(zkt_ctx* c);
bool msm_defers_tails(const zkt_ctx* c);
bool msm_batches_grouping(const zkt_ctx* c);

int lagrange_ensure(zkt_ctx* c, int log_n);
bool lagrange_ready(const zkt_ctx* c, int log_n);
size_t lagrange_bases(const zkt_ctx* c);
struct WireElimKeys {
    const void* pk[5];
    const size_t* pi_pos;
    size_t n_pi;
};
int wire_bases_prepare(zkt_ctx* c, int log_n, const uint32_t* const* d_idx, size_t n_rows, size_t n_vars, const WireElimKeys* elim = nullptr);
bool wire_bases_use(const zkt_ctx* c, int k);
int wire_bases_route(const zkt_ctx* c, int k);
int wire_bases_digest(zkt_ctx* c, const uint32_t* const* d_idx, size_t n_rows);
int wire_bases_lens(zkt_ctx* c, const uint32_t* d_lens);
int wire_bases_scalars(zkt_ctx* c, int k, const void* d_vars, const void* d_blinders, size_t n, const void** out, size_t* len);
bool wire_bases_check(zkt_ctx* c, int k, size_t n);
void wire_bases_drop(zkt_ctx* c);

}
```

zkt-plonk_amd/csrc/poly.hip:

```cpp
#include "poly.hpp"
#include "hostinv.hpp"

namespace zkt {

template <class P>
ZKT_D Fe<P> arg_fe(const uint32_t* w) {
    Fe<P> r;
#pragma unroll
    for (int i = 0; i < 8; ++i) r.v[i] = w[i];
    return r;
}

template <class P>
__global__ void k_mul_vec(const Fe<P>* a, const Fe<P>* b, Fe<P>* o, size_t n) {
    size_t i = (size_t)blockIdx.x * blockDim.x + threadIdx.x;
    if (i < n) fe_store<P>(o + i, fe_mul<P>(fe_load<P>(a + i), fe_load<P>(b + i)));
}

template <class P>
__global__ void k_trim_len(const Fe<P>* p, size_t lo, size_t n, uint32_t* len, int skip_if_set, Fe<P>* zero_at,
                           int zero_count) {
    if (zero_at && blockIdx.x == 0 && (int)threadIdx.x < zero_count) fe_store<P>(zero_at + threadIdx.x, fe_zero<P>());
    if (skip_if_set && *len != 0) return;
    size_t i = lo + (size_t)blockIdx.x * blockDim.x + threadIdx.x;
// ... 319 lines not shown
        if (li < n) fe_store<P>(out + (DEN ? n - 1 - li : li), t > 0 ? fe_mul<P>(pre, x[e]) : x[e]);
    }
    if (t == 255) fe_store<P>(totals + blockIdx.x, s[255]);
}
template <class P, int WHICH>
__global__ __launch_bounds__(256) void k_z_terms_scan(ZTermsArgs a, Fe<P>* pn, Fe<P>* sd, Fe<P>* tot_n, Fe<P>* tot_d) {
    __shared__ Fe<P> s[256];
    if (blockIdx.y) z_terms_scan<P, WHICH, true>(a, sd, tot_d, s);
    else z_terms_scan<P, WHICH, false>(a, pn, tot_n, s);
}

template <class P>
__global__ __launch_bounds__(256) void k_z_apply_combine(const Fe<P>* pn, const Fe<P>* sd, const Fe<P>* pre_n, const Fe<P>* pre_d,
                                                         Fe<P> inv_total, Fe<P>* out, size_t n) {
    const size_t b = blockIdx.x, rb = gridDim.x - 1 - b;
    Fe<P> k = inv_total;
    if (b) k = fe_mul<P>(k, fe_load<P>(pre_n + b - 1));
    if (rb) k = fe_mul<P>(k, fe_load<P>(pre_d + rb - 1));
#pragma unroll
    for (int e = 0; e < SC_E; ++e) {
        const size_t i = b * SC_BLK + (size_t)e * 256 + threadIdx.x;
        if (i >= n) break;
        Fe<P> v = fe_mul<P>(fe_load<P>(sd + i), k);
        if (i % SC_BLK) v = fe_mul<P>(v, fe_load<P>(pn + i - 1));
        fe_store<P>(out + i, v);
    }
}

constexpr int TB_THREADS = 1024;
template <class P>
ZKT_D uint32_t wg_trim_len(const Fe<P>* p, size_t n, uint32_t* best) {
    const int t = threadIdx.x;
    __syncthreads();
    if (t == 0) *best = 0;
    __syncthreads();
    for (size_t hi = n; hi > 0;) {
        const size_t lo = hi > (size_t)TB_THREADS ? hi - TB_THREADS : 0;
        const size_t i = lo + t;
        uint32_t v = 0;
        if (i < hi && !fe_is_zero<P>(fe_load<P>(p + i))) v = (uint32_t)(i + 1);
#pragma unroll
        for (int d = 32; d >= 1; d >>= 1) {
            uint32_t o = __shfl_down(v, d);
            v = o > v ? o : v;
        }
        if ((t & 63) == 0 && v) atomicMax(best, v);
        __syncthreads();
        const uint32_t found = *best;
        __syncthreads();
        if (found) return found;
        hi = lo;
    }
    return 0;
}
struct TrimBlindJob {
    void* poly;
    const void* bl;
    uint32_t* len;
    int k;
};
struct TrimBlindArgs {
    TrimBlindJob job[NTT_MAX_BATCH];
};
template <class P>
__global__ __launch_bounds__(TB_THREADS) void k_trim_blind(TrimBlindArgs a, size_t n, int zero_count) {
    __shared__ uint32_t best;
    const TrimBlindJob j = a.job[blockIdx.x];
    Fe<P>* p = (Fe<P>*)j.poly;
    const int t = threadIdx.x;
    if (t < zero_count) fe_store<P>(p + n + t, fe_zero<P>());
    if (j.k < 0) return;
    const uint32_t L = wg_trim_len<P>(p, n, &best);
    if (t == 0) *j.len = L;
    Fe<P> b = fe_zero<P>();
    if (t < j.k) {
        b = fe_load<P>((const Fe<P>*)j.bl + t);
        fe_store<P>(p + L + t, b);
    }
    __syncthreads();
    if (t < j.k) fe_store<P>(p + t, fe_sub<P>(fe_load<P>(p + t), b));
}

template <class P>
__global__ void k_lagrange_scalars(const Fe<P>* ev, size_t n, const uint32_t* len, const Fe<P>* bl, int k, const Fe<P>* roots,
                                   Fe<P> ninv, Fe<P>* D) {
    const size_t i = (size_t)blockIdx.x * blockDim.x + threadIdx.x;
    if (i >= n + (size_t)k) return;
    const size_t L = k ? (size_t)*len : n;
    if (i >= n) {
        const size_t t = i - n;
        Fe<P> acc = fe_zero<P>();
        for (int j = 0; j < k; ++j)
            if (L + j == n + t) acc = fe_add<P>(acc, fe_load<P>(bl + j));
        fe_store<P>(D + i, acc);
        return;
    }
    Fe<P> e0 = fe_load<P>(ev + i), e1 = (i + 1 < n) ? fe_load<P>(ev + i + 1) : fe_zero<P>();
    if (L != n) {
        for (int j = 0; j < k; ++j) {
            const size_t q = (L + j) & (n - 1);
            if (q == (size_t)j) continue;
            const Fe<P> b = fe_load<P>(bl + j);
            e0 = fe_add<P>(e0, fe_mul<P>(b, fe_sub<P>(fe_load<P>(roots + ((i * q) & (n - 1))), fe_load<P>(roots + ((i * j) & (n - 1))))));
            if (i + 1 < n)
                e1 = fe_add<P>(e1, fe_mul<P>(b, fe_sub<P>(fe_load<P>(roots + (((i + 1) * q) & (n - 1))),
                                                           fe_load<P>(roots + (((i + 1) * j) & (n - 1))))));
        }
    }
    fe_store<P>(D + i, fe_mul<P>(fe_sub<P>(e0, e1), ninv));
}

struct FxArg {
    uint32_t l[9];
};
struct QuotientDev {
    const void *a, *b, *c, *pi, *z1, *z2, *t, *h1, *h2;
    const void *q_m, *q_l, *q_r, *q_o, *q_c, *q_lookup, *q_table, *sigma1, *sigma2, *sigma3, *x, *l1;
    void* out;
    FxArg beta, delta, alpha_k3, alpha2, alpha3_opd_k2, alpha3_k2, alpha4, alpha5;
    FxArg gamma, epsilon, eopd;
    FxArg zh_inv[4];
    uint64_t n4;
    uint64_t first, count;
    const uint32_t* pi_tab;
    uint32_t n_pi_direct;
    uint32_t G, cls, next_off;
    const void *z1_next, *z2_next, *t_next, *h1_next;
    uint64_t cls_stride;
};
template <class P>
ZKT_D Fx<P> arg_fx(const FxArg& w) {
    Fx<P> r;
#pragma unroll
    for (int i = 0; i < FxP<P>::L; ++i) r.l[i] = w.l[i];
    return r;
}

template <class P>
__global__ __launch_bounds__(256) void k_quotient(QuotientDev q) {
    static_assert(FxP<P>::L == 9, "scalar field limbs");
    typedef Fx<P> X;
    const uint64_t i = q.first + (uint64_t)blockIdx.x * blockDim.x + threadIdx.x;
    if (i >= q.first + q.count) return;
    const uint64_t j = (i + q.next_off < q.n4) ? i + q.next_off : i + q.next_off - q.n4;
    const uint64_t coff = (uint64_t)blockIdx.y * q.cls_stride;
    const uint32_t cls = q.cls + blockIdx.y;
#define LD(ptr, idx) fx_unpack<P>(fe_load<P>((const Fe<P>*)(ptr) + coff + (idx)))
    const X beta = arg_fx<P>(q.beta), delta = arg_fx<P>(q.delta), gamma = arg_fx<P>(q.gamma);
    const X a = LD(q.a, i), b = LD(q.b, i), c = LD(q.c, i);
    X acc = fx_mul2_inl<P>(fx_mul<P>(a, b), LD(q.q_m, i), c, LD(q.q_o, i));
    acc = fx_add<P>(acc, fx_mul2_inl<P>(a, LD(q.q_l, i), b, LD(q.q_r, i)));
    const X l1 = LD(q.l1, i);
    if (q.pi_tab) {
        X pi = fx_zero<P>();
#pragma unroll 1
        for (uint32_t e = 0; e < q.n_pi_direct; e += 2) {
            X v[2], l[2];
#pragma unroll
            for (int h = 0; h < 2; ++h) {
                const uint32_t* ent = q.pi_tab + (size_t)(e + h) * 10;
                const bool live = e + h < q.n_pi_direct;
                const uint64_t rot = live ? ent[0] : 0;
                const uint64_t at = (i >= rot) ? i - rot : i + q.n4 - rot;
                l[h] = LD(q.l1, at);
#pragma unroll
                for (int w = 0; w < 9; ++w) v[h].l[w] = live ? ent[1 + w] : 0u;
            }
            pi = fx_add<P>(pi, fx_mul2_inl<P>(v[0], l[0], v[1], l[1]));
        }
        acc = fx_add<P>(acc, fx_add<P>(LD(q.q_c, i), pi));
    } else {
        acc = fx_add<P>(acc, fx_add<P>(LD(q.q_c, i), LD(q.pi, i)));
    }
    const X z1 = LD(q.z1, i), z1n = LD(q.z1_next, j);
    const X ag = fx_add<P>(a, gamma), bg = fx_add<P>(b, gamma), cg = fx_add<P>(c, gamma);
    const X one = fx_const_to_ark<P>();
    {
        const X bx = fx_mul<P>(LD(q.x, i), beta);
        const X d2 = fx_dbl<P>(bx), d4 = fx_dbl<P>(d2), d8 = fx_dbl<P>(d4);
        const X ak3 = arg_fx<P>(q.alpha_k3);
        X p1 = fx_mul<P>(z1, ak3);
        p1 = fx_mul<P>(p1, fx_add<P>(bx, ag));
        p1 = fx_mul<P>(p1, fx_add<P>(fx_sub<P, 2>(d8, bx), bg));
        X p2 = fx_mul<P>(z1n, ak3);
        p2 = fx_mul<P>(p2, fx_add<P>(fx_mul<P>(LD(q.sigma1, i), beta), ag));
        p2 = fx_mul<P>(p2, fx_add<P>(fx_mul<P>(LD(q.sigma2, i), beta), bg));
        const X p12 = fx_mul2_inl<P>(p1, fx_add<P>(fx_add<P>(fx_add<P>(d8, d4), bx), cg), fx_sub_lazy<P, 3>(fx_zero<P>(), p2),
                                     fx_add<P>(fx_mul<P>(LD(q.sigma3, i), beta), cg));
        acc = fx_add<P>(acc, p12);
    }
    {
        const X eps = arg_fx<P>(q.epsilon), eopd = arg_fx<P>(q.eopd);
// ... 449 lines not shown
    hipLaunchKernelGGL(k_z2_terms<P>, dim3(nblocks(a.n)), dim3(256), 0, c->stream, a);
    ZKT_HIP(c, hipGetLastError());
    return ZKT_OK;
}
int z2_terms(zkt_ctx* c, const ZTermsArgs& a) { ZKT_DISPATCH(c, z2_terms_t, a); }

template <class P> static int scan_mul_t(zkt_ctx* c, const void* in, void* out, size_t n, bool rev, void* tmp) {
    return scan_t<P, OpMul>(c, (const Fe<P>*)in, (Fe<P>*)out, n, rev, (Fe<P>*)tmp);
}
int scan_mul(zkt_ctx* c, const void* in, void* out, size_t n, bool reverse, void* d_tmp) { ZKT_DISPATCH(c, scan_mul_t, in, out, n, reverse, d_tmp); }
template <class P> static int scan_add_t(zkt_ctx* c, const void* in, void* out, size_t n, bool rev, void* tmp) {
    return scan_t<P, OpAdd>(c, (const Fe<P>*)in, (Fe<P>*)out, n, rev, (Fe<P>*)tmp);
}
int scan_add(zkt_ctx* c, const void* in, void* out, size_t n, bool reverse, void* d_tmp) { ZKT_DISPATCH(c, scan_add_t, in, out, n, reverse, d_tmp); }

template <class P> static int z_combine_t(zkt_ctx* c, const void* pn, const void* sd, const uint32_t* inv, void* out, size_t n) {
    hipLaunchKernelGGL(k_z_combine<P>, dim3(nblocks(n)), dim3(256), 0, c->stream, (const Fe<P>*)pn, (const Fe<P>*)sd, host_fe<P>(inv), (Fe<P>*)out, n);
    ZKT_HIP(c, hipGetLastError());
    return ZKT_OK;
}
int z_combine(zkt_ctx* c, const void* pn, const void* sd, const uint32_t inv_total[8], void* out, size_t n) { ZKT_DISPATCH(c, z_combine_t, pn, sd, inv_total, out, n); }

static size_t scan_tmp_elems(size_t n) {
    size_t nb = (n + SC_BLK - 1) / SC_BLK, need = 1;
    while (nb > 1) {
        need += 2 * nb;
        nb = (nb + SC_BLK - 1) / SC_BLK;
    }
    return need;
}
size_t grand_product_tmp_elems(size_t n) { return 2 * scan_tmp_elems(n); }
template <class P> static int grand_product_scan_t(zkt_ctx* c, const ZTermsArgs& a, int which, void* pn, void* sd, void* tmp,
                                                   const void** d_total_den, bool totals_later) {
    const size_t n = a.n;
    if (n == 0 || (n & (n - 1))) return set_err(c, ZKT_ERR_INVALID_ARGUMENT, "grand product: n must be a power of two");
    const size_t nb = (n + SC_BLK - 1) / SC_BLK;
    Fe<P>* tn = (Fe<P>*)tmp;
    Fe<P>* td = tn + scan_tmp_elems(n);
    if (which == 1)
        hipLaunchKernelGGL((k_z_terms_scan<P, 1>), dim3((unsigned)nb, 2), dim3(256), 0, c->stream, a, (Fe<P>*)pn, (Fe<P>*)sd, tn, td);
    else
        hipLaunchKernelGGL((k_z_terms_scan<P, 2>), dim3((unsigned)nb, 2), dim3(256), 0, c->stream, a, (Fe<P>*)pn, (Fe<P>*)sd, tn, td);
    ZKT_HIP(c, hipGetLastError());
    if (nb > 1 && !totals_later) {
        int rc;
        if ((rc = scan_t<P, OpMul>(c, tn, tn + nb, nb, false, tn + 2 * nb))) return rc;
        if ((rc = scan_t<P, OpMul>(c, td, td + nb, nb, false, td + 2 * nb))) return rc;
    }
    *d_total_den = nb > 1 ? td + nb + (nb - 1) : td;
    return ZKT_OK;
}
int grand_product_scan(zkt_ctx* c, const ZTermsArgs& a, int which, void* pn_local, void* sd_local, void* d_tmp, const void** d_total_den,
                       bool totals_later) {
    ZKT_DISPATCH(c, grand_product_scan_t, a, which, pn_local, sd_local, d_tmp, d_total_den, totals_later);
}
bool grand_product_totals_fit(size_t n) { return (n + SC_BLK - 1) / SC_BLK <= (size_t)SC_BLK; }
template <class P> static int grand_product_totals2_t(zkt_ctx* c, size_t n, void* tmp1, void* tmp2) {
    const size_t nb = (n + SC_BLK - 1) / SC_BLK;
    if (nb <= 1) return ZKT_OK;
    if (nb > (size_t)SC_BLK) return set_err(c, ZKT_ERR_INVALID_ARGUMENT, "grand product: the block totals need more than one block");
    Fe<P>*tn1 = (Fe<P>*)tmp1, *tn2 = (Fe<P>*)tmp2;
    hipLaunchKernelGGL((k_scan_rows4<P, OpMul>), dim3(1, 4), dim3(256), 0, c->stream, tn1, tn1 + scan_tmp_elems(n), tn2,
                       tn2 + scan_tmp_elems(n), nb);
    ZKT_HIP(c, hipGetLastError());
    return ZKT_OK;
}
int grand_product_totals2(zkt_ctx* c, size_t n, void* d_tmp1, void* d_tmp2) { ZKT_DISPATCH(c, grand_product_totals2_t, n, d_tmp1, d_tmp2); }
template <class P> static int grand_product_combine_t(zkt_ctx* c, const void* pn, const void* sd, const void* tmp, const uint32_t* inv,
                                                      void* out, size_t n) {
    const size_t nb = (n + SC_BLK - 1) / SC_BLK;
    const Fe<P>* tn = (const Fe<P>*)tmp;
    const Fe<P>* td = tn + scan_tmp_elems(n);
    hipLaunchKernelGGL(k_z_apply_combine<P>, dim3((unsigned)nb), dim3(256), 0, c->stream, (const Fe<P>*)pn, (const Fe<P>*)sd, tn + nb, td + nb,
                       host_fe<P>(inv), (Fe<P>*)out, n);
    ZKT_HIP(c, hipGetLastError());
    return ZKT_OK;
}
int grand_product_combine(zkt_ctx* c, const void* pn_local, const void* sd_local, const void* d_tmp, const uint32_t inv_total[8], void* out,
                          size_t n) {
    ZKT_DISPATCH(c, grand_product_combine_t, pn_local, sd_local, d_tmp, inv_total, out, n);
}

template <class P> static int lagrange_scalars_t(zkt_ctx* c, const void* ev, size_t n, const uint32_t* d_len, const void* d_bl, int k,
                                                 const void* roots, void* out) {
    Fe<P> nn = fe_zero<P>();
    nn.v[0] = (uint32_t)(n & 0xffffffffu);
    nn.v[1] = (uint32_t)((uint64_t)n >> 32);
    const Fe<P> ninv = fe_inv_host<P>(fe_to_mont<P>(nn));
    hipLaunchKernelGGL(k_lagrange_scalars<P>, dim3(nblocks(n + (size_t)k)), dim3(256), 0, c->stream, (const Fe<P>*)ev, n, d_len,
                       (const Fe<P>*)d_bl, k, (const Fe<P>*)roots, ninv, (Fe<P>*)out);
    ZKT_HIP(c, hipGetLastError());
    return ZKT_OK;
}
int lagrange_scalars(zkt_ctx* c, const void* ev, size_t n, const uint32_t* d_len, const void* d_blinders, int k, const void* d_roots,
                     void* out) {
    ZKT_DISPATCH(c, lagrange_scalars_t, ev, n, d_len, d_blinders, k, d_roots, out);
}

template <class P> static FxArg hat_arg(const Fe<P>& s) {
    const Fx<P> h = fx_cond_sub_p<P>(fx_from_ark<P>(s));
    FxArg r;
    for (int i = 0; i < 9; ++i) r.l[i] = h.l[i];
    return r;
}
template <class P> static FxArg ark_arg(const Fe<P>& s) {
    const Fx<P> h = fx_unpack<P>(s);
    FxArg r;
    for (int i = 0; i < 9; ++i) r.l[i] = h.l[i];
    return r;
}
template <class P> static int quotient_t(zkt_ctx* c, const QuotientArgs& a) {
    ProfScope prof(c, "quotient");
    auto get = [](const uint32_t* w) { Fe<P> r; for (int i = 0; i < 8; ++i) r.v[i] = w[i]; return r; };
    const Fe<P> alpha = get(a.alpha), beta = get(a.beta), gamma = get(a.gamma), delta = get(a.delta), eps = get(a.epsilon);
    const Fe<P> k2 = fe_from_u32<P>(1u << 10), k3 = fe_from_u32<P>(1u << 15);
    const Fe<P> a2 = fe_sqr<P>(alpha), a3 = fe_mul<P>(a2, alpha), a4 = fe_mul<P>(a3, alpha), a5 = fe_mul<P>(a4, alpha);
    const Fe<P> opd = fe_add<P>(delta, fe_one<P>());
    QuotientDev q{};
    q.a = a.a; q.b = a.b; q.c = a.c; q.pi = a.pi; q.z1 = a.z1; q.z2 = a.z2; q.t = a.t; q.h1 = a.h1; q.h2 = a.h2;
    q.q_m = a.q_m; q.q_l = a.q_l; q.q_r = a.q_r; q.q_o = a.q_o; q.q_c = a.q_c; q.q_lookup = a.q_lookup; q.q_table = a.q_table;
    q.sigma1 = a.sigma1; q.sigma2 = a.sigma2; q.sigma3 = a.sigma3; q.x = a.x; q.l1 = a.l1; q.out = a.out;
    q.beta = hat_arg<P>(beta);
    q.delta = hat_arg<P>(delta);
    q.alpha_k3 = hat_arg<P>(fe_mul<P>(alpha, k3));
    q.alpha2 = hat_arg<P>(a2);
    q.alpha3_opd_k2 = hat_arg<P>(fe_mul<P>(fe_mul<P>(a3, opd), k2));
    q.alpha3_k2 = hat_arg<P>(fe_mul<P>(a3, k2));
    q.alpha4 = hat_arg<P>(a4);
    q.alpha5 = hat_arg<P>(a5);
    q.gamma = ark_arg<P>(gamma);
    q.epsilon = ark_arg<P>(eps);
    q.eopd = ark_arg<P>(fe_mul<P>(eps, opd));
    for (int k = 0; k < 4; ++k) q.zh_inv[k] = hat_arg<P>(get(a.zh_inv[k]));
    q.n4 = a.n4;
    q.pi_tab = a.pi_tab;
    q.n_pi_direct = a.n_pi_direct;
    if (a.G <= 1) {
        q.G = 1; q.cls = 0; q.next_off = 4;
        q.z1_next = a.z1; q.z2_next = a.z2; q.t_next = a.t; q.h1_next = a.h1;
    } else {
        q.G = a.G; q.cls = a.cls; q.next_off = a.next_off;
        q.z1_next = a.z1_next; q.z2_next = a.z2_next; q.t_next = a.t_next; q.h1_next = a.h1_next;
    }
    if (a.pi_tab && a.n_pi_direct > (uint32_t)QUOTIENT_PI_DIRECT_MAX)
        return set_err(c, ZKT_ERR_INVALID_ARGUMENT, "too many direct public inputs");
    q.first = a.first;
    q.count = a.count ? a.count : a.n4 - a.first;
    if (q.first + q.count > a.n4) return set_err(c, ZKT_ERR_INVALID_ARGUMENT, "quotient range outside the vectors");
    const unsigned ncls = a.ncls > 1 ? a.ncls : 1;
    if (ncls > 1 && (a.G <= 1 || a.cls + ncls > a.G)) return set_err(c, ZKT_ERR_INVALID_ARGUMENT, "quotient classes outside the coset");
    q.cls_stride = ncls > 1 ? a.cls_stride : 0;
    hipLaunchKernelGGL(k_quotient<P>, dim3(nblocks(q.count), ncls), dim3(256), 0, c->stream, q);
    ZKT_HIP(c, hipGetLastError());
    return ZKT_OK;
}
template <class P> static int to_hat_t(zkt_ctx* c, void* v, size_t n, int k32) {
    if (k32 == 0) hipLaunchKernelGGL((k_to_hat<P, 0>), dim3(nblocks(n)), dim3(256), 0, c->stream, (Fe<P>*)v, n);
    else hipLaunchKernelGGL((k_to_hat<P, 1>), dim3(nblocks(n)), dim3(256), 0, c->stream, (Fe<P>*)v, n);
    ZKT_HIP(c, hipGetLastError());
    return ZKT_OK;
}
int to_hat_form(zkt_ctx* c, void* v, size_t n, int k32) { ZKT_DISPATCH(c, to_hat_t, v, n, k32); }
int quotient_pointwise(zkt_ctx* c, const QuotientArgs& a) { ZKT_DISPATCH(c, quotient_t, a); }

template <class P>
__global__ void k_interleave(const Fe<P>* in, Fe<P>* out, uint64_t n4, uint32_t log_g, uint64_t piece) {
    const uint64_t t = (uint64_t)blockIdx.x * blockDim.x + threadIdx.x;
    if (t >= n4) return;
    const uint64_t cls = t & ((1u << log_g) - 1), i = t >> log_g;
    const uint64_t j = i / piece, o = i - j * piece;
    fe_store<P>(out + t, fe_load<P>(in + ((j << log_g) + cls) * piece + o));
}
template <class P> static int interleave_t(zkt_ctx* c, const void* in, void* out, size_t n4, uint32_t G, uint32_t chunks) {
    uint32_t lg = 0;
    while ((1u << lg) < G) ++lg;
    const uint64_t m = n4 >> lg;
    if (chunks == 0 || m % chunks) return set_err(c, ZKT_ERR_INVALID_ARGUMENT, "interleave: pieces must divide the class");
    hipLaunchKernelGGL(k_interleave<P>, dim3(nblocks(n4)), dim3(256), 0, c->stream, (const Fe<P>*)in, (Fe<P>*)out, (uint64_t)n4, lg,
                       m / chunks);
// ... 299 lines not shown
```

zkt-plonk_amd/csrc/poly.hpp:

```cpp
#pragma once
#include "ctx.hpp"

namespace zkt {

constexpr int LC_MAX_TERMS = 24;
struct LinCombArgs {
    const void* poly[LC_MAX_TERMS];
    uint64_t len[LC_MAX_TERMS];
    uint32_t scalar[LC_MAX_TERMS][8];
    int nterms;
};

constexpr int EVAL_MAX = 16;
struct EvalArgs {
    const void* poly[EVAL_MAX];
    uint64_t len[EVAL_MAX];
    uint32_t point[EVAL_MAX][8];
    int count;
    uint8_t table[EVAL_MAX];
};

struct QuotientArgs {
    const void *a, *b, *c, *pi, *z1, *z2, *t, *h1, *h2;
    const void *q_m, *q_l, *q_r, *q_o, *q_c, *q_lookup, *q_table, *sigma1, *sigma2, *sigma3, *x, *l1;
    void* out;
    uint32_t alpha[8], beta[8], gamma[8], delta[8], epsilon[8];
    uint32_t zh_inv[4][8];
    uint64_t n4;
    const uint32_t* pi_tab;
    uint32_t n_pi_direct;
    uint32_t G, cls, next_off;
    const void *z1_next, *z2_next, *t_next, *h1_next;
    uint64_t first, count;
    uint32_t ncls;
    uint64_t cls_stride;
};
constexpr int QUOTIENT_PI_DIRECT_MAX = 16;

struct ZTermsArgs {
    const void *a, *b, *c, *s1, *s2, *s3, *roots;
    const void *f, *t, *h1, *h2;
    void *num, *den;
    uint32_t beta[8], gamma[8], delta[8], epsilon[8];
    uint64_t n;
};

int poly_mul_vec(zkt_ctx* c, const void* a, const void* b, void* out, size_t n);
int poly_set_zero(zkt_ctx* c, void* p, size_t n_elems);
int poly_trim_len(zkt_ctx* c, const void* p, size_t n, uint32_t* d_len, void* zero_at = nullptr, int zero_count = 0);
int poly_copy_pad(zkt_ctx* c, const void* d_in, size_t len, void* out, size_t n);
int poly_gather_pad(zkt_ctx* c, const void* d_values, size_t n_vars, const uint32_t* d_idx, size_t rows, void* out, size_t n,
                    uint32_t* d_status);
int poly_add_blinders(zkt_ctx* c, void* p, const uint32_t* d_len, const void* d_blinders, int k, size_t cap);
int poly_lincomb(zkt_ctx* c, const LinCombArgs& a, void* out, size_t n);
struct TrimBlindSpec {
    void* poly;
    const void* d_blinders;
    uint32_t* d_len;
    int k;
};
int poly_trim_blind(zkt_ctx* c, const TrimBlindSpec* jobs, int nb, size_t n, int zero_count);
int lagrange_scalars(zkt_ctx* c, const void* ev, size_t n, const uint32_t* d_len, const void* d_blinders, int k, const void* d_roots,
                     void* out);
int poly_eval_many(zkt_ctx* c, const EvalArgs& a, void* d_partials, void* d_results, void* d_powers);
int poly_eval_open_tables(zkt_ctx* c, const EvalArgs& a, const uint32_t z0[8], const uint32_t z0_inv[8], const uint32_t z1[8],
                          const uint32_t z1_inv[8], size_t len, void* d_partials, void* d_results, void* d_powers);
int z1_terms(zkt_ctx* c, const ZTermsArgs& a);
int z2_terms(zkt_ctx* c, const ZTermsArgs& a);
int scan_mul(zkt_ctx* c, const void* in, void* out, size_t n, bool reverse, void* d_tmp );
int scan_add(zkt_ctx* c, const void* in, void* out, size_t n, bool reverse, void* d_tmp);
int z_combine(zkt_ctx* c, const void* pn, const void* sd, const uint32_t inv_total[8], void* out, size_t n);
size_t grand_product_tmp_elems(size_t n);
int grand_product_scan(zkt_ctx* c, const ZTermsArgs& a, int which, void* pn_local, void* sd_local, void* d_tmp, const void** d_total_den,
                       bool totals_later = false);
bool grand_product_totals_fit(size_t n);
int grand_product_totals2(zkt_ctx* c, size_t n, void* d_tmp1, void* d_tmp2);
int grand_product_combine(zkt_ctx* c, const void* pn_local, const void* sd_local, const void* d_tmp, const uint32_t inv_total[8], void* out,
                          size_t n);
int quotient_pointwise(zkt_ctx* c, const QuotientArgs& a);
int to_hat_form(zkt_ctx* c, void* v, size_t n, int k32);
int quotient_interleave(zkt_ctx* c, const void* in, void* out, size_t n4, uint32_t G, uint32_t chunks = 1);
int quotient_split_blind(zkt_ctx* c, const void* q, size_t n, const void* d_b0b1, void* q_lo, void* q_mid, void* q_hi,
                         uint32_t* d_status, bool fused = false, bool closed = false);
constexpr int QC_WIN = 14, QC_WIN_POLYS = 6;
int quotient_classes_of_coset(zkt_ctx* c, const void* in, void* out, size_t n);
int quotient_gather_windows(zkt_ctx* c, const void* const* polys, size_t first, void* out);
int quotient_classes_combine(zkt_ctx* c, void* q, size_t n, const uint32_t* vinv, const uint32_t* u, const uint32_t* g3);
int quotient_classes_close(zkt_ctx* c, void* q, size_t n, const uint32_t* vinv, const uint32_t* u, const uint32_t* g3, void* q_lo,
                           void* q_mid, void* q_hi);
int open_witness(zkt_ctx* c, const void* p, size_t len, const uint32_t z[8], const uint32_t z_inv[8], void* d_tmp_a, void* d_tmp_b,
                 void* d_scan_tmp, void* out, void* d_powers );
size_t open_witness_powers(size_t maxlen);
constexpr int OPEN_PW_ROW = 257;
int open_elems(size_t len);
size_t open_blocks(size_t len);
int open_pow_tables(zkt_ctx* c, const uint32_t z[8], const uint32_t z_inv[8], void* d_powers, size_t len);
int open_divide(zkt_ctx* c, const void* t, size_t len, void* d_tmp, void* d_scan_tmp, void* out, const void* d_powers,
                void* d_total = nullptr);
int open_combine(zkt_ctx* c, const LinCombArgs& a, void* out, size_t len, const void* d_powers);
int poly_sum_rows(zkt_ctx* c, const void* d_partials, int nblk, int rows, void* d_out);
int sigma_build(zkt_ctx* c, int log_n, const uint32_t* d_w_l, const uint32_t* d_w_r, const uint32_t* d_w_o, size_t n_rows, size_t n_vars,
                void* const* d_sigma);
size_t sigma_scratch_bytes(int log_n, size_t n_rows);
int sigma_enqueue(zkt_ctx* c, int log_n, const uint32_t* d_w_l, const uint32_t* d_w_r, const uint32_t* d_w_o, size_t n_rows, size_t n_vars,
                  void* const* d_sigma, void* d_scratch, uint32_t* d_flag);
struct WitnessCheckKeys {
    int log_n;
    const void* pk[5];
    const void* q_lookup_ev;
    const void* sigma_ev[3];
};
int selector_evals_enqueue(zkt_ctx* c, int log_n, const void* const* pk, void* const* outs);
int witness_check(zkt_ctx* c, const WitnessCheckKeys& keys, const zkt_prove_inputs& in, int flags, zkt_witness_report* out);
struct WitnessPlanKeys {
    int log_n;
    const void* pk[5];
};
int witness_plan_create(zkt_ctx* c, const WitnessPlanKeys& keys, const uint32_t* w_l, const uint32_t* w_r, const uint32_t* w_o,
                        size_t n_rows, size_t n_vars, int wiring_on_device, const size_t* pi_pos, size_t n_pi, uint32_t rules,
                        zkt_witness_plan** out);
int witness_check_batch(zkt_ctx* c, const WitnessCheckKeys& keys, const zkt_witness_batch& in, int flags, zkt_witness_report* out);
int gen_powers(zkt_ctx* c, void* out, size_t n, const uint32_t base[8], const uint32_t scale[8]);
int lookup_count(zkt_ctx* c, const void* f, size_t n, const void* d_sorted_keys, const uint32_t* d_perm, uint32_t nkeys,
                 uint32_t* d_counts, uint32_t* d_status);
int lookup_starts(zkt_ctx* c, const uint32_t* d_base_counts, uint32_t* d_hits, uint32_t nkeys, size_t n, uint32_t* d_even,
                  uint32_t* d_odd, uint32_t* d_status);
int lookup_expand(zkt_ctx* c, const void* d_keys_insertion, const uint32_t* d_starts, uint32_t nkeys, void* out, size_t n);

}
```

zkt-plonk_amd/csrc/prover.hip:

```cpp
#include "circuit.hpp"
#include <chrono>
#include <cstdio>
#include <cstdlib>
#include "linearisation.hpp"
#include "msm.hpp"
#include "transcript.hpp"

#include <algorithm>
#include <functional>
#include <cstring>
#include <memory>
#include <optional>
#include <vector>

namespace zkt {

template <class Q>
static void serialize_point(const Affine<Q>& p, std::vector<uint8_t>& out) {
    const size_t nb = Q::N * 4;
    std::vector<uint8_t> b(nb, 0);
    if (aff_is_inf<Q>(p)) {
        b[nb - 1] |= 0x40;
    } else {
        fq_to_le<Q>(p.x, b.data());
// ... 39 lines not shown
    void dump_marks() {
        if (!trace_on || marks.empty()) return;
        for (size_t i = 1; i < marks.size(); ++i)
            fprintf(stderr, "[zkt host] %-28s %8.1f us\n", marks[i].first,
                    std::chrono::duration<double, std::micro>(marks[i].second - marks[i - 1].second).count());
        marks.clear();
    }

    void tr_commit(const char* label, const Affine<Q>& p) {
        uint8_t x[64], y[64];
        bool inf = aff_is_inf<Q>(p);
        if (!inf) {
            fq_to_le<Q>(p.x, x);
            fq_to_le<Q>(p.y, y);
        }
        tr.append_commitment(label, x, y, Q::N * 4, inf);
    }
    void tr_scalar(const char* label, const F& v) {
        uint8_t b[32];
        H::to_le_bytes(v, b);
        tr.append_scalars(label, b, 1, 32, true);
    }
    F tr_challenge(const char* label) {
        uint8_t b[32];
        tr.challenge_scalar(label, R::BITS, b);
        return H::from_le_bytes(b);
    }
    static void put(uint32_t dst[8], const F& v) { memcpy(dst, v.v, 32); }

    std::optional<ProfScope> idle;
    void wait_begin() {
        if (c->prof_on && !idle) idle.emplace(c, "host_wait");
    }
    void wait_end() { idle.reset(); }

    int commit_begin(const void* d_poly, size_t len, int slot) {
        if (!c->sharded()) return msm_begin(c, d_poly, len, 0, 1, slot);
        size_t off, cnt, total;
        msm_slice(c, &off, &cnt, &total);
        if (len > total)
            return set_err(c, ZKT_ERR_TOO_MANY_COEFFICIENTS, "TooManyCoefficients: polynomial longer than the committer key");
        S.have[slot] = len > off;
        if (!S.have[slot]) return ZKT_OK;
        const size_t l = std::min(len, off + cnt) - off;
        return msm_begin(c, (const char*)d_poly + off * 32, l, 0, 1, slot);
    }
    struct Pending {
        const void* scalars;
        size_t len;
        int slot, tbl;
    };
    Pending queue[6];
    int n_queue = 0, n_lag_queued = 0;
    bool queueing() const { return !c->sharded() && !c->batch_off && msm_batches_grouping(c); }
    int commit_flush() {
        const int k = n_queue;
        const void* sc[6];
        size_t lens[6];
        int slots[6], tbls[6];
        for (int j = 0; j < k; ++j) {
            sc[j] = queue[j].scalars; lens[j] = queue[j].len; slots[j] = queue[j].slot; tbls[j] = queue[j].tbl;
        }
        n_queue = 0;
        n_lag_queued = 0;
        return msm_begin_many(c, k, sc, lens, 1, slots, tbls, true);
    }
    int commit_push(const void* scalars, size_t len, int slot, int tbl) {
        if (n_queue == 6)
            if (int rc = commit_flush()) return rc;
        queue[n_queue++] = Pending{scalars, len, slot, tbl};
        return ZKT_OK;
    }
    int commit_begin_many(void* const* d_polys, const size_t* lens, const int* slots, int k) {
        for (int j = 0; j < k; ++j) {
            const int rc = queueing() ? commit_push(d_polys[j], lens[j], slots[j], 0) : commit_begin(d_polys[j], lens[j], slots[j]);
            if (rc) return rc;
        }
        return ZKT_OK;
    }
    int commit_evals_begin(const void* ev, const void* d_poly, int blinder_off, int k, int len_slot, int slot) {
        const bool q = queueing();
        if (!lagrange_ready(c, S.log_n) || c->lagrange_off)
            return q ? commit_push(d_poly, S.n + (size_t)k, slot, 0) : commit_begin(d_poly, S.n + (size_t)k, slot);
        if (q && n_lag_queued == 3)
            if (int rc0 = commit_flush()) return rc0;
        void* d = q ? S.lag_scalars_q[n_lag_queued] : S.lag_scalars;
        int rc = lagrange_scalars(c, ev, S.n, S.status + 8 + len_slot, (const char*)S.small + (size_t)blinder_off * 32, k, S.roots, d);
        if (rc) return rc;
        if (!q) return msm_begin(c, d, S.n + (size_t)k, 0, 1, slot, 1);
        ++n_lag_queued;
        return commit_push(d, S.n + (size_t)k, slot, 1);
    }
    int commit_collect(const int* slots, const bool* skip, int k, Affine<Q>* out) {
        wait_begin();
        if (!c->sharded()) {
            for (int j = 0; j < k; ++j) {
                if (skip && skip[j]) continue;
                uint64_t xy[12];
                int rc = msm_end(c, slots[j], xy);
                if (rc) return rc;
                memcpy(out[j].x.v, xy, Q::N * 4);
                memcpy(out[j].y.v, xy + Q::N / 2, Q::N * 4);
            }
            return ZKT_OK;
        }
        bool have[16];
        uint64_t xy[16 * 12];
        for (int j = 0; j < k; ++j) have[j] = !(skip && skip[j]) && S.have[slots[j]];
        int rc = msm_end_sharded(c, slots, have, k, xy);
        if (rc) return rc;
        for (int j = 0; j < k; ++j) {
            if (skip && skip[j]) continue;
            memcpy(out[j].x.v, xy + 12 * j, Q::N * 4);
            memcpy(out[j].y.v, xy + 12 * j + Q::N / 2, Q::N * 4);
        }
        return ZKT_OK;
    }

    int collect_wires(Affine<Q>* cm, int* took = nullptr) {
        for (int k = 0; k < 3; ++k) {
            const bool routed = S.wire_route[k];
            S.wire_route[k] = false;
            if (took) took[k] = 0;
            if (!routed) continue;
            if (wire_bases_check(c, k, S.n)) {
                if (took) took[k] = wire_bases_route(c, k);
                continue;
            }
            static const int slot[1] = {0};
            int rc = msm_begin(c, S.poly[k], S.n + 2, 0, 1, 0);
            if (rc || (rc = commit_collect(slot, nullptr, 1, cm + k))) return rc;
        }
        return ZKT_OK;
    }

    struct PolyJob {
        const void* ev;
        void* poly;
        int blinder_off, k, len_slot;
    };
    int evals_to_blinded_polys(const PolyJob* jobs, int nb) {
        const size_t n = S.n;
        int rc;
        const void* ins[NTT_MAX_BATCH];
        void* outs[NTT_MAX_BATCH];
        size_t lens[NTT_MAX_BATCH];
        for (int y = 0; y < nb; ++y) {
            ins[y] = jobs[y].ev;
            outs[y] = jobs[y].poly;
            lens[y] = n;
        }
        if ((rc = ntt_run_batch(c, S.log_n, 1, 0, nb, ins, lens, outs))) return rc;
        if (c->fused(4)) {
            TrimBlindSpec tb[NTT_MAX_BATCH];
            for (int y = 0; y < nb; ++y)
                tb[y] = TrimBlindSpec{jobs[y].poly, (const char*)S.small + (size_t)jobs[y].blinder_off * 32, S.status + 8 + jobs[y].len_slot,
                                      jobs[y].k > 0 ? jobs[y].k : -1};
            return poly_trim_blind(c, tb, nb, n, 8);
        }
        for (int y = 0; y < nb; ++y) {
            void* poly = jobs[y].poly;
            if (jobs[y].k > 0) {
                if ((rc = poly_trim_len(c, poly, n, S.status + 8 + jobs[y].len_slot, (char*)poly + n * 32, 8))) return rc;
                if ((rc = poly_add_blinders(c, poly, S.status + 8 + jobs[y].len_slot,
                                            (const char*)S.small + (size_t)jobs[y].blinder_off * 32, jobs[y].k, n + 8)))
                    return rc;
            } else {
                ZKT_HIP(c, hipMemsetAsync((char*)poly + n * 32, 0, 8 * 32, c->stream));
            }
        }
        return ZKT_OK;
    }
    int evals_to_blinded_poly(const void* ev, void* poly, int blinder_off, int k, int len_slot) {
        const PolyJob j{ev, poly, blinder_off, k, len_slot};
        return evals_to_blinded_polys(&j, 1);
    }

    int check_status() {
        uint32_t st = 0;
        ZKT_HIP(c, hipMemcpyAsync(&st, S.status, 4, hipMemcpyDeviceToHost, c->stream));
        wait_begin();
        ZKT_HIP(c, hipStreamSynchronize(c->stream));
        if (st & 16u) return set_err(c, ZKT_ERR_INVALID_ARGUMENT, "wire index outside the variable map");
// ... 1071 lines not shown
```

Baseline: 69.89 proofs/s.

## Add sparse Lagrange-basis commitment path compacting nonzero scalars before MSM

When the Lagrange table is in use and the MSM is large, the Lagrange scalar kernel now compacts nonzero scalars into a capped list through a wave-aggregated atomic append. A dedicated sparse MSM then computes digits only for those entries and sums bucket rows and columns directly. This is meant to avoid the full bucket-sort MSM for commitments whose evaluation vectors are mostly zero. If the count exceeds the cap, the path records an overflow, falls back to a dense MSM and marks that commitment kind dense for later proofs, so the first oversized attempt wastes some work.

```diff
diff --git a/include/zkt_plonk.h b/include/zkt_plonk.h
--- a/include/zkt_plonk.h
+++ b/include/zkt_plonk.h
@@ -98,6 +98,7 @@
                      uint64_t* out_w_xy_mont, int* out_w_is_infinity, uint64_t* out_evals_mont);
 
 int zkt_ctx_set_lagrange(zkt_ctx* ctx, int on);
+int zkt_ctx_set_sparse_commit(zkt_ctx* ctx, int mode);
 int zkt_ctx_set_wire_elimination(zkt_ctx* ctx, int mode);
 int zkt_ctx_set_quotient_route(zkt_ctx* ctx, int mode);
 int zkt_ctx_set_fused_passes(zkt_ctx* ctx, int mode);
diff --git a/zkt-plonk_amd/_lib.py b/zkt-plonk_amd/_lib.py
--- a/zkt-plonk_amd/_lib.py
+++ b/zkt-plonk_amd/_lib.py
@@ -1749,6 +1749,10 @@
         self._L.zkt_ctx_set_lagrange.argtypes = [ctypes.c_void_p, ctypes.c_int]
         self.check(self._L.zkt_ctx_set_lagrange(self._h, int(on)))
 
+    def set_sparse_commit(self, mode: int = 0):
+        self._L.zkt_ctx_set_sparse_commit.argtypes = [ctypes.c_void_p, ctypes.c_int]
+        self.check(self._L.zkt_ctx_set_sparse_commit(self._h, int(mode)))
+
     def set_wire_elimination(self, mode: int = 1):
         self._L.zkt_ctx_set_wire_elimination.argtypes = [ctypes.c_void_p, ctypes.c_int]
         self.check(self._L.zkt_ctx_set_wire_elimination(self._h, int(mode)))
diff --git a/zkt-plonk_amd/csrc/capi.hip b/zkt-plonk_amd/csrc/capi.hip
--- a/zkt-plonk_amd/csrc/capi.hip
+++ b/zkt-plonk_amd/csrc/capi.hip
@@ -269,6 +269,7 @@
     (void)hipStreamSynchronize(parent->stream);
     c->is_fork = true;
     c->lagrange_off = parent->lagrange_off;
+    c->sparse_commit_mode = parent->sparse_commit_mode;
     c->wire_elim_mode = parent->wire_elim_mode;
     c->quotient_route = parent->quotient_route;
     c->fused_passes = parent->fused_passes;
@@ -356,6 +357,14 @@
 int zkt_ctx_set_lagrange(zkt_ctx* c, int on) {
     if (!c) return ZKT_ERR_INVALID_ARGUMENT;
     c->lagrange_off = !on;
+    ++c->msm_epoch;
+    return ZKT_OK;
+}
+
+int zkt_ctx_set_sparse_commit(zkt_ctx* c, int mode) {
+    if (!c) return ZKT_ERR_INVALID_ARGUMENT;
+    if (mode < 0 || mode > 2) return set_err(c, ZKT_ERR_INVALID_ARGUMENT, "mode: 0 automatic, 1 wherever the Lagrange table serves, 2 off");
+    c->sparse_commit_mode = mode;
     ++c->msm_epoch;
     return ZKT_OK;
 }
diff --git a/zkt-plonk_amd/csrc/circuit.hpp b/zkt-plonk_amd/csrc/circuit.hpp
--- a/zkt-plonk_amd/csrc/circuit.hpp
+++ b/zkt-plonk_amd/csrc/circuit.hpp
@@ -79,6 +79,12 @@
     uint64_t t_srs_generation = 0;
     uint64_t t_commit_xy[12] = {};
     bool wire_route[3] = {};
+    struct SparseFallback {
+        const void* poly = nullptr;
+        size_t len = 0;
+        int kind = -1;
+    } sparse_fb[16];
+    bool sparse_dense[5] = {};
     bool wire_dense_only = false;
     int wire_elim_force = -1;
     bool use_classes = false;
diff --git a/zkt-plonk_amd/csrc/circuit_steps.hip b/zkt-plonk_amd/csrc/circuit_steps.hip
--- a/zkt-plonk_amd/csrc/circuit_steps.hip
+++ b/zkt-plonk_amd/csrc/circuit_steps.hip
@@ -96,10 +96,22 @@
         if (k && (rc = poly_add_blinders(c, poly, d_len, d_bl, k, n + 8))) return rc;
     }
     if (path == 0) return msm_g1_dev(c, poly, n + (size_t)k, 0, 1, out_xy, out_is_infinity);
-    if ((rc = lagrange_scalars(c, d_evals, n, d_len, d_bl, k, S.roots, S.lag_scalars))) return rc;
-    if ((rc = msm_begin(c, S.lag_scalars, n + (size_t)k, 0, 1, 0, 1))) return rc;
     uint64_t xy[12] = {};
-    if ((rc = msm_end(c, 0, xy))) return rc;
+    bool overflow = false;
+    if (msm_sparse_wanted(c) && !S.sparse_dense[4]) {
+        MsmSparseList sp;
+        if ((rc = msm_sparse_prepare(c, 0, &sp))) return rc;
+        if ((rc = lagrange_scalars(c, d_evals, n, d_len, d_bl, k, S.roots, S.lag_scalars, &sp))) return rc;
+        if ((rc = msm_sparse_begin(c, 0)) || (rc = msm_end(c, 0, xy, &overflow))) return rc;
+        if (overflow) {
+            S.sparse_dense[4] = true;
+            if ((rc = msm_begin(c, poly, n + (size_t)k, 0, 1, 0)) || (rc = msm_end(c, 0, xy))) return rc;
+        }
+    } else {
+        if ((rc = lagrange_scalars(c, d_evals, n, d_len, d_bl, k, S.roots, S.lag_scalars))) return rc;
+        if ((rc = msm_begin(c, S.lag_scalars, n + (size_t)k, 0, 1, 0, 1))) return rc;
+        if ((rc = msm_end(c, 0, xy))) return rc;
+    }
     const size_t words = c->curve == ZKT_CURVE_BN254 ? 8 : 12;
     memcpy(out_xy, xy, words * 8);
     if (out_is_infinity) {
diff --git a/zkt-plonk_amd/csrc/ctx.hpp b/zkt-plonk_amd/csrc/ctx.hpp
--- a/zkt-plonk_amd/csrc/ctx.hpp
+++ b/zkt-plonk_amd/csrc/ctx.hpp
@@ -88,6 +88,7 @@
     bool aux_off = false;
     bool batch_off = false;
     bool lagrange_off = false;
+    int sparse_commit_mode = 0;
     int wire_elim_mode = 1;
     int quotient_route = 0;
     int verify_terms_mode = 0;
diff --git a/zkt-plonk_amd/csrc/msm.hip b/zkt-plonk_amd/csrc/msm.hip
--- a/zkt-plonk_amd/csrc/msm.hip
+++ b/zkt-plonk_amd/csrc/msm.hip
@@ -826,6 +826,103 @@
     if (lane == 0) xx_store_ark<Q>(partials + y, acc);
 }
 
+template <class C, int DIG>
+__global__ __launch_bounds__(256) void k_msm_sparse_digits(const uint32_t* ctl, const uint32_t* pos, const Fe<typename C::Fr>* scalars,
+                                                           uint32_t cap, MsmWindows win, uint64_t tcount, uint64_t base_off,
+                                                           uint2* entries) {
+    using R = typename C::Fr;
+    if (ctl[1]) return;
+    const uint32_t cnt = ctl[0] < cap ? ctl[0] : cap;
+    const uint32_t r = blockIdx.x * blockDim.x + threadIdx.x;
+    if (r >= cnt) return;
+    const Fe<R> s = fe_load<R>(scalars + r);
+    const uint32_t p = pos[r];
+    uint2* out = entries + (size_t)r * (uint32_t)win.W;
+    msm_for_each_digit_sel<R, DIG>(s, win, [&](int w, uint32_t d, uint32_t neg) {
+        out[w] = make_uint2((uint32_t)((size_t)w * tcount + base_off + p) | (neg << 31), d);
+    });
+}
+template <class C>
+static auto msm_pick_sparse_digits(int dig) -> decltype(&k_msm_sparse_digits<C, 0>) {
+    switch (dig) {
+        case 1: return k_msm_sparse_digits<C, 1>;
+        case 2: return k_msm_sparse_digits<C, 2>;
+        case 3: return k_msm_sparse_digits<C, 3>;
+        case 4: return k_msm_sparse_digits<C, 4>;
+        case 5: return k_msm_sparse_digits<C, 5>;
+        default: return k_msm_sparse_digits<C, 0>;
+    }
+}
+
+constexpr uint32_t MSM_SPARSE_QUEUE = 128;
+template <class C, bool MSM_TAIL_INL>
+__global__ __launch_bounds__(256) void k_msm_sparse_sums(uint32_t q1, uint32_t q2, uint32_t B, uint32_t W, uint32_t cap,
+                                                         const uint32_t* ctl, const uint2* entries,
+                                                         const Affine<typename C::Fq>* table, Xyzz<typename C::Fq>* rowcol,
+                                                         Xyzz<typename C::Fq>* top, uint32_t* overflow_out) {
+    using Q = typename C::Fq;
+    __shared__ uint32_t queue[4][MSM_SPARSE_QUEUE];
+    const uint32_t NI = 1u << q1, NJ = 1u << q2;
+    const uint32_t lane = threadIdx.x & 63u, wv = threadIdx.x >> 6;
+    const uint32_t w = blockIdx.x * 4u + wv;
+    const uint32_t over = ctl[1];
+    if (blockIdx.x == 0 && threadIdx.x == 0) *overflow_out = over;
+    if (over || w > NI + NJ) return;
+    const uint32_t cnt = ctl[0] < cap ? ctl[0] : cap;
+    const uint32_t total = cnt * W;
+    volatile uint32_t* qv = queue[wv];
+    uint32_t qn = 0;
+    XyzzX<Q> acc = xx_identity<Q>();
+    auto add_queued = [&](uint32_t take) {
+        if (lane >= take) return;
+        const uint32_t v = qv[lane];
+        const Affine<Q>* pt = table + (v & 0x7fffffffu);
+        const Fe<Q> cx = fe_load<Q>(&pt->x), cy = fe_load<Q>(&pt->y);
+        if (fe_is_zero<Q>(cx) && fe_is_zero<Q>(cy)) return;
+        AffineX<Q> q;
+        q.x = fx_unpack<Q>(cx);
+        q.y = fx_unpack<Q>(cy);
+        if (v >> 31) q.y = fx_sub<Q, 1>(fx_zero<Q>(), q.y);
+        acc = xx_add_mixed<Q, true>(acc, q);
+    };
+    auto load4 = [&](uint32_t base, uint2* e) {
+#pragma unroll
+        for (int k = 0; k < 4; ++k) {
+            const uint32_t i = base + 64u * k + lane;
+            e[k] = (base < total && i < total) ? entries[i] : make_uint2(0u, 0u);
+        }
+    };
+    uint2 cur[4], nxt[4];
+    load4(0, cur);
+    for (uint32_t base = 0; base < total; base += 256u) {
+        load4(base + 256u, nxt);
+#pragma unroll
+        for (int k = 0; k < 4; ++k) {
+            const uint32_t d = cur[k].y;
+            bool mine;
+            if (w < NI) mine = d != 0 && d < B && (d >> q2) == w;
+            else if (w < NI + NJ) mine = d != 0 && d < B && (d & (NJ - 1u)) == w - NI;
+            else mine = d == B;
+            const uint64_t bal = __ballot(mine);
+            if (bal == 0) continue;
+            if (mine) qv[qn + (uint32_t)__popcll(bal & ((1ull << lane) - 1ull))] = cur[k].x;
+            qn += (uint32_t)__popcll(bal);
+            if (qn >= 64u) {
+                add_queued(64u);
+                const uint32_t rem = qn - 64u;
+                const uint32_t t = lane < rem ? qv[64u + lane] : 0u;
+                if (lane < rem) qv[lane] = t;
+                qn = rem;
+            }
+        }
+#pragma unroll
+        for (int k = 0; k < 4; ++k) cur[k] = nxt[k];
+    }
+    add_queued(qn);
+    acc = wave_sum<Q, MSM_TAIL_INL>(acc);
+    if (lane == 0) xx_store<Q>(w < NI + NJ ? rowcol + w : top, acc);
+}
+
 template <class C>
 __global__ void k_srs_to_fx(Affine<typename C::Fq>* table, size_t total) {
     using Q = typename C::Fq;
@@ -839,6 +936,8 @@
 }
 
 static int msm_rows(int c) { return c - 1; }
+template <class Q>
+static constexpr size_t msm_overflow_offset() { return (size_t)(MSM_MAX_Y + 1) * MSM_R2_BLOCKS * sizeof(Xyzz<Q>); }
 
 template <class C, bool VB = false>
 static auto msm_pick_bin_count(int dig) -> decltype(&k_msm_bin_count<C, 0, VB>) {
@@ -1040,13 +1139,18 @@
             const int q = P.c - 1, q2 = q / 2, q1 = q - q2;
             if ((rc = st->work.alloc(c, &st->rowcol[i], (((size_t)1 << q1) + ((size_t)1 << q2)) * sizeof(Xyzz<Q>)))) return rc;
         }
-        if ((rc = st->work.pinned(c, &st->host_result[i], (size_t)(MSM_MAX_Y + 1) * MSM_R2_BLOCKS * sizeof(Xyzz<Q>), hipHostMallocMapped))) return rc;
+        if ((rc = st->work.pinned(c, &st->host_result[i], msm_overflow_offset<Q>() + 64, hipHostMallocMapped))) return rc;
+        memset((char*)st->host_result[i] + msm_overflow_offset<Q>(), 0, 64);
+        if ((rc = st->work.alloc(c, (void**)&st->sp_ctl[i], 16))) return rc;
+        if ((rc = st->work.alloc(c, &st->sp_list[i], (size_t)MSM_SPARSE_CAP_MAX * (sizeof(Fe<R>) + 4)))) return rc;
+        if ((rc = st->work.alloc(c, &st->sp_entries[i], (size_t)MSM_SPARSE_CAP_MAX * P.W * sizeof(uint2)))) return rc;
         ZKT_HIP(c, hipHostGetDevicePointer(&st->host_result_dev[i], st->host_result[i], 0));
         if ((rc = st->work.event(c, &st->ev_main[i]))) return rc;
         if ((rc = st->work.event(c, &st->ev_done[i]))) return rc;
     }
     st->defer_tails = count <= MSM_DEFER_MAX;
     if (const char* e = exp_env("ZKT_MSM_DEFER")) st->defer_tails = atoi(e) != 0;
+    if (const char* e = exp_env("ZKT_SPARSE_CAP")) st->sp_cap = std::min((uint32_t)std::max(atoi(e), 1), MSM_SPARSE_CAP_MAX);
     c->msm = st;
     ++c->msm_epoch;
     ++c->srs_generation;
@@ -1338,6 +1442,7 @@
         ZKT_HIP(c, hipEventRecord(st.ev_main[slots[j]], c->stream));
         st.tail_wait[st.n_tail_wait++] = slots[j];
         st.pending[slots[j]] = true;
+        st.sparse[slots[j]] = false;
         if (st.defer_tails && st.n_tail_wait < MSM_TAIL_BATCH) continue;
         if (int rc = msm_launch_tails<C>(c)) return rc;
     }
@@ -1359,14 +1464,102 @@
 }
 
 template <class C>
-static int msm_collect(zkt_ctx* c, int slot, Affine<typename C::Fq>* out) {
+static int msm_collect(zkt_ctx* c, int slot, Affine<typename C::Fq>* out, bool* overflow = nullptr) {
     using Q = typename C::Fq;
     MsmState& st = *c->msm;
     if (int rc0 = msm_launch_tails<C>(c)) return rc0;
     ZKT_HIP(c, hipEventSynchronize(st.ev_done[slot]));
     st.pending[slot] = false;
+    if (overflow) *overflow = false;
+    if (st.sparse[slot]) {
+        st.sparse[slot] = false;
+        if (*(const volatile uint32_t*)((const char*)st.host_result[slot] + msm_overflow_offset<Q>())) {
+            if (!overflow) return set_err(c, ZKT_ERR_INVALID_ARGUMENT, "sparse commitment overflowed and nobody takes it again");
+            *overflow = true;
+            out->x = fe_zero<Q>();
+            out->y = fe_zero<Q>();
+            return ZKT_OK;
+        }
+        if (c->prof_on == 1) ++c->prof["msm_sparse"].calls;
+    }
     *out = xyzz_to_affine_host<Q>(msm_host_finish<Q>(st, slot));
     return ZKT_OK;
+}
+
+template <class C>
+static int msm_sparse_prepare_t(zkt_ctx* c, int slot, MsmSparseList* out) {
+    MsmState& st = *c->msm;
+    ++c->msm_epoch;
+    for (int w = 0; w < st.n_tail_wait; ++w)
+        if (st.tail_wait[w] == slot)
+            if (int rc0 = msm_launch_tails<C>(c)) return rc0;
+    if (st.pending[slot]) ZKT_HIP(c, hipStreamWaitEvent(c->stream, st.ev_done[slot], 0));
+    ZKT_HIP(c, hipMemsetAsync(st.sp_ctl[slot], 0, 8, c->stream));
+    out->ctl = st.sp_ctl[slot];
+    out->pos = (uint32_t*)st.sp_list[slot];
+    out->scalars = (char*)st.sp_list[slot] + (size_t)MSM_SPARSE_CAP_MAX * 4;
+    out->cap = st.sp_cap;
+    return ZKT_OK;
+}
+template <class C, bool TI>
+static int msm_sparse_begin_t(zkt_ctx* c, int slot) {
+    using Q = typename C::Fq;
+    using R = typename C::Fr;
+    MsmState& st = *c->msm;
+    const MsmPlan& P = st.plan;
+    const uint32_t cap = st.sp_cap;
+    const uint32_t* pos = (const uint32_t*)st.sp_list[slot];
+    const Fe<R>* sc = (const Fe<R>*)((const char*)st.sp_list[slot] + (size_t)MSM_SPARSE_CAP_MAX * 4);
+    {
+        ProfScope prof_main(c, "msm_lag_main");
+        hipLaunchKernelGGL(msm_pick_sparse_digits<C>(P.dig), dim3((cap + 255) / 256), dim3(256), 0, c->stream, st.sp_ctl[slot], pos, sc,
+                           cap, P.win, (uint64_t)st.tbl_count(1), (uint64_t)0, (uint2*)st.sp_entries[slot]);
+        ZKT_HIP(c, hipGetLastError());
+    }
+    ZKT_HIP(c, hipEventRecord(st.ev_main[slot], c->stream));
+    ZKT_HIP(c, hipStreamWaitEvent(st.side, st.ev_main[slot], 0));
+    {
+        ProfScope prof_tail(c, "msm_tail", st.side);
+        const uint32_t q = (uint32_t)(P.c - 1), q2 = q / 2, q1 = q - q2;
+        const uint32_t sums = (1u << q1) + (1u << q2) + 1u;
+        hipLaunchKernelGGL((k_msm_sparse_sums<C, TI>), dim3((sums + 3) / 4), dim3(256), 0, st.side, q1, q2, P.Bw, (uint32_t)P.W, cap,
+                           st.sp_ctl[slot], (const uint2*)st.sp_entries[slot], (const Affine<Q>*)st.tbl_table(1),
+                           (Xyzz<Q>*)st.rowcol[slot], (Xyzz<Q>*)st.buckets[slot] + P.Bw,
+                           (uint32_t*)((char*)st.host_result_dev[slot] + msm_overflow_offset<Q>()));
+        ZKT_HIP(c, hipGetLastError());
+        MsmTailBatch tb{};
+        for (int j = 0; j < MSM_TAIL_BATCH; ++j) {
+            tb.buckets[j] = st.buckets[slot];
+            tb.rowcol[j] = st.rowcol[slot];
+            tb.partials[j] = st.host_result_dev[slot];
+        }
+        hipLaunchKernelGGL((k_msm_weighted_rows<C, TI>), dim3(q + 1, 1), dim3(64), 0, st.side, q1, q2, P.Bw, tb);
+        ZKT_HIP(c, hipGetLastError());
+    }
+    ZKT_HIP(c, hipEventRecord(st.ev_done[slot], st.side));
+    st.pending[slot] = true;
+    st.sparse[slot] = true;
+    return ZKT_OK;
+}
+int msm_sparse_prepare(zkt_ctx* c, int slot, MsmSparseList* out) {
+    if (!c->msm || !c->msm->table2) return set_err(c, ZKT_ERR_NOT_LOADED, "no Lagrange-basis table built");
+    if (slot < 0 || slot >= MsmState::SLOTS) return set_err(c, ZKT_ERR_INVALID_ARGUMENT, "bad MSM slot");
+    if (c->curve == ZKT_CURVE_BN254) return msm_sparse_prepare_t<Bn254Curve>(c, slot, out);
+    return msm_sparse_prepare_t<Bls381Curve>(c, slot, out);
+}
+int msm_sparse_begin(zkt_ctx* c, int slot) {
+    if (!c->msm || !c->msm->table2) return set_err(c, ZKT_ERR_NOT_LOADED, "no Lagrange-basis table built");
+    if (slot < 0 || slot >= MsmState::SLOTS) return set_err(c, ZKT_ERR_INVALID_ARGUMENT, "bad MSM slot");
+    bool inl = c->msm->defer_tails || c->msm->count <= MSM_TAIL_INL_MAX;
+    if (const char* e = exp_env("ZKT_MSM_TAIL_INL")) inl = atoi(e) != 0;
+    if (c->curve == ZKT_CURVE_BN254) return inl ? msm_sparse_begin_t<Bn254Curve, true>(c, slot) : msm_sparse_begin_t<Bn254Curve, false>(c, slot);
+    return inl ? msm_sparse_begin_t<Bls381Curve, true>(c, slot) : msm_sparse_begin_t<Bls381Curve, false>(c, slot);
+}
+bool msm_sparse_wanted(const zkt_ctx* c) {
+    if (!c->msm || !c->msm->table2 || c->sharded() || c->lagrange_off) return false;
+    if (c->sparse_commit_mode == 2) return false;
+    if (c->sparse_commit_mode == 1) return true;
+    return c->msm->count > ((size_t)1 << 17) + 64;
 }
 
 template <class C>
@@ -1470,17 +1663,17 @@
     }
     return msm_flush_tails(c);
 }
-int msm_end(zkt_ctx* c, int slot, uint64_t* out_xy) {
+int msm_end(zkt_ctx* c, int slot, uint64_t* out_xy, bool* overflow) {
     if (c->curve == ZKT_CURVE_BN254) {
         Affine<Bn254Fq> a;
-        int rc = msm_collect<Bn254Curve>(c, slot, &a);
+        int rc = msm_collect<Bn254Curve>(c, slot, &a, overflow);
         if (rc) return rc;
         memcpy(out_xy, a.x.v, 32);
         memcpy(out_xy + 4, a.y.v, 32);
         return ZKT_OK;
     }
     Affine<Bls381Fq> a;
-    int rc = msm_collect<Bls381Curve>(c, slot, &a);
+    int rc = msm_collect<Bls381Curve>(c, slot, &a, overflow);
     if (rc) return rc;
     memcpy(out_xy, a.x.v, 48);
     memcpy(out_xy + 6, a.y.v, 48);
diff --git a/zkt-plonk_amd/csrc/msm.hpp b/zkt-plonk_amd/csrc/msm.hpp
--- a/zkt-plonk_amd/csrc/msm.hpp
+++ b/zkt-plonk_amd/csrc/msm.hpp
@@ -53,6 +53,15 @@
     uint32_t* heavy[MSM_TAIL_BATCH];
     void* rowcol[MSM_TAIL_BATCH];
     void* partials[MSM_TAIL_BATCH];
+};
+
+constexpr uint32_t MSM_SPARSE_CAP = 2048;
+constexpr uint32_t MSM_SPARSE_CAP_MAX = 8192;
+struct MsmSparseList {
+    uint32_t* ctl = nullptr;
+    uint32_t* pos = nullptr;
+    void* scalars = nullptr;
+    uint32_t cap = 0;
 };
 
 constexpr int MSM_HEAVY = 32;
@@ -125,6 +134,11 @@
     hipStream_t side = nullptr;
     hipEvent_t ev_main[SLOTS] = {}, ev_done[SLOTS] = {};
     bool pending[SLOTS] = {};
+    uint32_t* sp_ctl[SLOTS] = {};
+    void* sp_list[SLOTS] = {};
+    void* sp_entries[SLOTS] = {};
+    uint32_t sp_cap = MSM_SPARSE_CAP;
+    bool sparse[SLOTS] = {};
     bool defer_tails = false;
     int tail_wait[SLOTS] = {};
     int n_tail_wait = 0;
@@ -161,7 +175,10 @@
 int msm_begin_batch(zkt_ctx* c, int k, const void* const* d_scalars, const size_t* ns, int mont, const int* slots, const int* tbls);
 int msm_begin_many(zkt_ctx* c, int k, const void* const* d_scalars, const size_t* ns, int mont, const int* slots, const int* tbls,
                    bool grouped, const std::function<int(int)>& ready = {});
-int msm_end(zkt_ctx* c, int slot, uint64_t* out_xy);
+int msm_end(zkt_ctx* c, int slot, uint64_t* out_xy, bool* overflow = nullptr);
+int msm_sparse_prepare(zkt_ctx* c, int slot, MsmSparseList* out);
+int msm_sparse_begin(zkt_ctx* c, int slot);
+bool msm_sparse_wanted(const zkt_ctx* c);
 int msm_end_sharded(zkt_ctx* c, const int* slots, const bool* have, int k, uint64_t* out_xy );
 int msm_flush_tails(zkt_ctx* c);
 bool msm_defers_tails(const zkt_ctx* c);
diff --git a/zkt-plonk_amd/csrc/poly.hip b/zkt-plonk_amd/csrc/poly.hip
--- a/zkt-plonk_amd/csrc/poly.hip
+++ b/zkt-plonk_amd/csrc/poly.hip
@@ -425,8 +425,26 @@
 }
 
 template <class P>
+ZKT_D void lagrange_append(const Fe<P>& d, size_t i, MsmSparseList sp) {
+    const bool nz = !fe_is_zero<P>(d);
+    const uint64_t bal = __ballot(nz);
+    if (!nz) return;
+    const uint32_t lane = threadIdx.x & 63u;
+    const int leader = __ffsll((long long)bal) - 1;
+    uint32_t base = 0;
+    if ((int)lane == leader) base = atomicAdd(sp.ctl, (uint32_t)__popcll(bal));
+    base = __shfl(base, leader);
+    const uint32_t at = base + (uint32_t)__popcll(bal & ((1ull << lane) - 1ull));
+    if (at < sp.cap) {
+        sp.pos[at] = (uint32_t)i;
+        fe_store<P>((Fe<P>*)sp.scalars + at, d);
+    } else {
+        sp.ctl[1] = 1u;
+    }
+}
+template <class P, bool SPARSE>
 __global__ void k_lagrange_scalars(const Fe<P>* ev, size_t n, const uint32_t* len, const Fe<P>* bl, int k, const Fe<P>* roots,
-                                   Fe<P> ninv, Fe<P>* D) {
+                                   Fe<P> ninv, Fe<P>* D, MsmSparseList sp) {
     const size_t i = (size_t)blockIdx.x * blockDim.x + threadIdx.x;
     if (i >= n + (size_t)k) return;
     const size_t L = k ? (size_t)*len : n;
@@ -436,6 +454,7 @@
         for (int j = 0; j < k; ++j)
             if (L + j == n + t) acc = fe_add<P>(acc, fe_load<P>(bl + j));
         fe_store<P>(D + i, acc);
+        if (SPARSE) lagrange_append<P>(acc, i, sp);
         return;
     }
     Fe<P> e0 = fe_load<P>(ev + i), e1 = (i + 1 < n) ? fe_load<P>(ev + i + 1) : fe_zero<P>();
@@ -450,7 +469,9 @@
                                                            fe_load<P>(roots + (((i + 1) * j) & (n - 1))))));
         }
     }
-    fe_store<P>(D + i, fe_mul<P>(fe_sub<P>(e0, e1), ninv));
+    const Fe<P> d = fe_mul<P>(fe_sub<P>(e0, e1), ninv);
+    fe_store<P>(D + i, d);
+    if (SPARSE) lagrange_append<P>(d, i, sp);
 }
 
 struct FxArg {
@@ -1066,19 +1087,20 @@
 }
 
 template <class P> static int lagrange_scalars_t(zkt_ctx* c, const void* ev, size_t n, const uint32_t* d_len, const void* d_bl, int k,
-                                                 const void* roots, void* out) {
+                                                 const void* roots, void* out, const MsmSparseList* sparse) {
     Fe<P> nn = fe_zero<P>();
     nn.v[0] = (uint32_t)(n & 0xffffffffu);
     nn.v[1] = (uint32_t)((uint64_t)n >> 32);
     const Fe<P> ninv = fe_inv_host<P>(fe_to_mont<P>(nn));
-    hipLaunchKernelGGL(k_lagrange_scalars<P>, dim3(nblocks(n + (size_t)k)), dim3(256), 0, c->stream, (const Fe<P>*)ev, n, d_len,
-                       (const Fe<P>*)d_bl, k, (const Fe<P>*)roots, ninv, (Fe<P>*)out);
+    auto kern = sparse ? k_lagrange_scalars<P, true> : k_lagrange_scalars<P, false>;
+    hipLaunchKernelGGL(kern, dim3(nblocks(n + (size_t)k)), dim3(256), 0, c->stream, (const Fe<P>*)ev, n, d_len,
+                       (const Fe<P>*)d_bl, k, (const Fe<P>*)roots, ninv, (Fe<P>*)out, sparse ? *sparse : MsmSparseList{});
     ZKT_HIP(c, hipGetLastError());
     return ZKT_OK;
 }
 int lagrange_scalars(zkt_ctx* c, const void* ev, size_t n, const uint32_t* d_len, const void* d_blinders, int k, const void* d_roots,
-                     void* out) {
-    ZKT_DISPATCH(c, lagrange_scalars_t, ev, n, d_len, d_blinders, k, d_roots, out);
+                     void* out, const MsmSparseList* sparse) {
+    ZKT_DISPATCH(c, lagrange_scalars_t, ev, n, d_len, d_blinders, k, d_roots, out, sparse);
 }
 
 template <class P> static FxArg hat_arg(const Fe<P>& s) {
diff --git a/zkt-plonk_amd/csrc/poly.hpp b/zkt-plonk_amd/csrc/poly.hpp
--- a/zkt-plonk_amd/csrc/poly.hpp
+++ b/zkt-plonk_amd/csrc/poly.hpp
@@ -1,5 +1,6 @@
 #pragma once
 #include "ctx.hpp"
+#include "msm.hpp"
 
 namespace zkt {
 
@@ -61,7 +62,7 @@
 };
 int poly_trim_blind(zkt_ctx* c, const TrimBlindSpec* jobs, int nb, size_t n, int zero_count);
 int lagrange_scalars(zkt_ctx* c, const void* ev, size_t n, const uint32_t* d_len, const void* d_blinders, int k, const void* d_roots,
-                     void* out);
+                     void* out, const MsmSparseList* sparse = nullptr);
 int poly_eval_many(zkt_ctx* c, const EvalArgs& a, void* d_partials, void* d_results, void* d_powers);
 int poly_eval_open_tables(zkt_ctx* c, const EvalArgs& a, const uint32_t z0[8], const uint32_t z0_inv[8], const uint32_t z1[8],
                           const uint32_t z1_inv[8], size_t len, void* d_partials, void* d_results, void* d_powers);
diff --git a/zkt-plonk_amd/csrc/prover.hip b/zkt-plonk_amd/csrc/prover.hip
--- a/zkt-plonk_amd/csrc/prover.hip
+++ b/zkt-plonk_amd/csrc/prover.hip
@@ -145,6 +145,18 @@
         const bool q = queueing();
         if (!lagrange_ready(c, S.log_n) || c->lagrange_off)
             return q ? commit_push(d_poly, S.n + (size_t)k, slot, 0) : commit_begin(d_poly, S.n + (size_t)k, slot);
+        const int kind = len_slot == 3 ? 0 : len_slot == 4 ? 1 : len_slot == 5 ? 2 : 3;
+        if (msm_sparse_wanted(c) && !S.sparse_dense[kind]) {
+            MsmSparseList sp;
+            int rc = msm_sparse_prepare(c, slot, &sp);
+            if (rc || (rc = lagrange_scalars(c, ev, S.n, S.status + 8 + len_slot, (const char*)S.small + (size_t)blinder_off * 32, k,
+                                             S.roots, S.lag_scalars, &sp)))
+                return rc;
+            S.sparse_fb[slot].poly = d_poly;
+            S.sparse_fb[slot].len = S.n + (size_t)k;
+            S.sparse_fb[slot].kind = kind;
+            return msm_sparse_begin(c, slot);
+        }
         if (q && n_lag_queued == 3)
             if (int rc0 = commit_flush()) return rc0;
         void* d = q ? S.lag_scalars_q[n_lag_queued] : S.lag_scalars;
@@ -160,8 +172,15 @@
             for (int j = 0; j < k; ++j) {
                 if (skip && skip[j]) continue;
                 uint64_t xy[12];
-                int rc = msm_end(c, slots[j], xy);
+                bool overflow = false;
+                int rc = msm_end(c, slots[j], xy, &overflow);
                 if (rc) return rc;
+                if (overflow) {
+                    const CircuitState::SparseFallback fb = S.sparse_fb[slots[j]];
+                    if (fb.kind < 0) return set_err(c, ZKT_ERR_INVALID_ARGUMENT, "sparse commitment without a fallback");
+                    S.sparse_dense[fb.kind] = true;
+                    if ((rc = commit_begin(fb.poly, fb.len, slots[j])) || (rc = msm_end(c, slots[j], xy))) return rc;
+                }
                 memcpy(out[j].x.v, xy, Q::N * 4);
                 memcpy(out[j].y.v, xy + Q::N / 2, Q::N * 4);
             }
```

Result: slower. 68.47 proofs/s (-2.0%).
